# apache/yunikorn-k8shim

Measured on AMD Instinct MI355X. Metric: pod×node predicate evals/sec + decisions/sec, 50k nodes × 1M pods, higher is better.
Workload: dtype int64; 1 GPU; configs[2]: 50k nodes x 1M pods, NodeResourcesFit + TaintToleration + NodeAffinity; nodes_per_gpu=50000, total_nodes=50000, pods=1000000, templates=2000, pod_classes=2061, signature_planes=327, unique_requests=False, spread=False, gang_size=0, parallelism=single GPU

## Files before the change

yunikorn-k8shim_amd/csrc/engine/engine.hip:

```cpp
#include "../../../include/ykpred.h"

#include <hip/hip_runtime.h>
#include <dlfcn.h>
#include <rccl/rccl.h>

#include <algorithm>
#include <chrono>
#include <cstdio>
#include <cstdlib>
#include <cstring>
#include <mutex>
#include <string>
#include <map>
#include <unordered_map>
#include <vector>

#include "kernels.hip.h"
#include "ask_tasks.h"
#include "preempt_headroom_finish.h"

using ykk::i64;
using ykk::u64;

namespace {
// ... 205 lines not shown
  std::vector<int32_t> h_row_big;
  std::vector<int32_t> h_sorted_off;
  DevBuf d_sorted, d_sorted_off, d_ent_c;
  int sweep_min_run = 1;
  int sweep_groups = 0;
  bool sweep_ready = false;
  std::vector<int32_t> h_class_sweep;
  int sweep_rows[ykk::kMaxIdxRows] = {0, 0}, sweep_row_off[ykk::kMaxIdxRows + 1] = {0, 0, 0}, sweep_runs = 0;
  int index_rows_needed = 0;
  DevBuf d_agree;
  DevBuf d_query;
  DevBuf d_groups;
  DevBuf d_domain_head;
  DevBuf d_rc_req, d_rc_pods, d_rc_ports;
  int rc_tiers = 0;
  bool rc_ports = false;
  DevBuf d_vt_base, d_vt_tier_end, d_vt_cum, d_vt_ports;
  std::vector<int32_t> h_vt_base, h_vt_cap;
  int vt_tiers = 0;
  size_t vt_rows = 0;
  bool vt_ports = false;
  int64_t vt_max_cap = 0;
  DevBuf d_pround;
  DevBuf d_vfx_col, d_vfx_cum;
  int vfx_columns = -1;
  std::vector<uint8_t> vfx_stale;
  int64_t vfx_stale_nodes = 0;
  DevBuf d_pround_live;
  DevBuf d_bytes_gather;
  DevBuf d_topo_agree;
  u64 dict_digest = 0;
  int fuse_rows = 1;
  int fuse_wpl = 0;
  int fuse_count = 0, fuse_row_count = 0;
  bool fuse_ready = false;
  DevBuf d_fuse_rec;
  int fuse_combos = 0;
  int fuse_combine = 1;
  DevBuf d_fuse_combo_rec, d_fuse_combo;
  std::vector<uint8_t> h_class_fused;
  int run_decide = 1;
  int run_ranges = 0, n_decide_list = 0, run_decide_classes = -1;
  bool win_partial = false;
  DevBuf d_run_ranges, d_no_decide, d_glin_r;
  int class_runs = 1;
  int class_runs_min_rows = 16;
  int run_classes = 0, run_units = 0, run_rows = 0;
  DevBuf d_run_classes, d_run_units;
  DevBuf d_sweep_rows, d_sweep_runs, d_sweep_units;
  int sweep_units[ykk::kMaxIdxRows] = {0, 0}, sweep_unit_off[ykk::kMaxIdxRows + 1] = {0, 0, 0};
  DevBuf d_chunk_list_b0;
  int NCB0 = 0;
  DevBuf d_walk2_order, d_walk2_big, d_walk2_begin, d_walk2_len;
  int walk2_chunks = -1;
  DevBuf d_first_r;
  static constexpr bool decide_skip = true;
  DevBuf d_chunk_list_b;
  DevBuf d_slice_general;
  DevBuf d_slice_desc;
  DevBuf d_pfx_r;
  DevBuf d_idx_c;
  DevBuf d_win_r;
  int idx_stride = 0;
  DevBuf d_sig_tol, d_sig_tolflags, d_sig_ports, d_swanted;
  DevBuf d_sig_aff_flags, d_sig_aff_off, d_sig_aff_terms, d_sig_pre_off, d_sig_pre_terms;
  bool specs_set = false;

  int P = 0, C = 0, NC = 0;
  std::vector<int32_t> h_pod_spec, h_pod_pin;
  DevBuf d_pod_spec, d_pod_pin, d_pod_class;
  DevBuf d_class_sig, d_class_pin, d_class_first, d_class_word, d_chunk_class, d_chunk_begin, d_chunk_len, d_chunk_first, d_members;
  std::unordered_map<ClassKey, int32_t, ClassKeyHash> class_ids;
  std::vector<int32_t> h_pod_class, h_pod_slot;
  std::vector<int32_t> h_pod_row;
  int rows_total = 0, rows_a = 0, row_capacity = 0;
  DevBuf d_pod_row;
  bool bands_enabled = true;
  int band_steps = 0;
  int band_steps_now = 128;
  int round_batched = -1;
  int round_node_assume = 1;
  int round_prof = 0;
  int fail_after = 0;
  int sig_wpl = 0;
  int combine_slices = 1;
  int decide_groups_from = 16384;
  int early_counts = 1;
  int group_lds = -1;
  int group_scratch_mb = 256;
  int affinity_fill_waves = 0;
  int group_chunk_tasks = 0;
  int max_lds_bytes = 64 * 1024;
  int num_cus = 256;
  int n_bands = 0, n_band_steps = 0, n_classes_a = 0, n_fix_rows = 0;
  std::vector<int32_t> h_class_slot_a;
  DevBuf d_band_tab, d_class_rows_a, d_class_list_a, d_class_slot_a, d_fix_row, d_fix_slot, d_chunk_zone;
  DevBuf d_class_list_b;
  int n_classes_b = 0;
  std::vector<int32_t> h_ch_zone;
  std::vector<uint8_t> h_row_stale;
  std::vector<int32_t> h_class_sig, h_class_pin, h_class_first, h_class_live;
  std::vector<std::vector<int32_t>> h_class_chunks;
  std::vector<int32_t> h_members, h_ch_class, h_ch_begin, h_ch_len, h_ch_first;
  int patch_chunks = 0;
  bool rank_valid = false;
  uint64_t specs_version = 1, ranked_specs_version = 0, ranked_nodes_epoch = 0;
  unsigned ranked_pre = 0, ranked_filt = 0;
  bool ranked_has_first = false;
  DevBuf d_round;
  DevBuf d_fx_off, d_fx_cls, d_fx_cnt, d_fx_occ, d_sp_sig_of;
  uint64_t fx_version = 0;
  bool fx_contrib = false, fx_ports = false;
  std::vector<int32_t> h_fx_off;
  std::vector<int32_t> h_fx_cls;
  std::vector<int32_t> h_fx_cnt;
  std::vector<uint8_t> h_fx_occupies;
  DevBuf d_patches, d_rows, d_row_count, d_row_best;
  unsigned last_pre = 0, last_filt = 0;
  bool last_eval_valid = false;
  DevBuf d_class_count, d_class_best;
  bool pods_set = false, classes_dirty = true;
  int chunk_members = ykk::kChunkMembers;
  bool chunk_sorted = true;
  int combine_lds_bytes = 40000;

  DevBuf d_bitmap, d_counts, d_decisions, d_keys, d_scratch;
  void* last_bitmap = nullptr;
  int64_t last_bitmap_rows = 0;
  void *last_counts = nullptr, *last_decisions = nullptr, *last_keys = nullptr;

  hipStream_t aux_stream = nullptr;
  hipEvent_t ev_fork = nullptr, ev_planes = nullptr, ev_join = nullptr, ev_counts = nullptr, ev_zero = nullptr;
  hipStream_t peek_stream = nullptr;
  hipEvent_t ev_eval_done = nullptr;
  void* peek_pinned = nullptr;
  size_t peek_pinned_bytes = 0;

  struct GraphKey {
    uint64_t version;
    unsigned pre, filt, options;
    void *bitmap, *counts, *decisions, *keys;
    bool operator==(const GraphKey& o) const {
      return version == o.version && pre == o.pre && filt == o.filt && options == o.options && bitmap == o.bitmap && counts == o.counts &&
             decisions == o.decisions && keys == o.keys;
    }
  };
  std::vector<std::pair<GraphKey, hipGraphExec_t>> graphs;
  std::vector<GraphKey> seen;
  uint64_t tables_version = 1;
  bool graph_disabled = true;

  ncclComm_t comm = nullptr;
  int comm_rank = 0, comm_world = 1, node_offset = 0;
  int64_t round_exchanges = 0;
  void* h_round_pinned = nullptr;
  size_t h_round_pinned_bytes = 0;
  int64_t rounds_batched = 0, round_batched_asks = 0, round_batches = 0, rounds_sequential = 0, round_sequential_asks = 0;
  int forced_stride = 0;
  DevBuf d_gathered, d_gathered_map, d_xkey, d_xcand;
  bool last_has_keys = false;
  DevBuf d_class_rows_all, d_gathered_classes, d_class_rows_slot, d_class_sig_ident, d_expand_count, d_layout_hash, d_gathered_pod_class, d_row_pod;
  int ident_classes = 0;
  uint64_t layout_version = 1, layout_hashed_version = 0, layout_hash_value = 0, row_pod_version = 0;
  uint64_t ask_epoch = 1, hdr_epoch = 0;
  std::vector<uint64_t> hdr_cache;
  uint64_t nodes_epoch = 1, hist_epoch = 0;
  uint64_t bitmap_epoch = 0;

  int64_t n_full_evals = 0, n_node_patches = 0, n_row_patches = 0, n_queries = 0, n_gathers = 0, n_uploads = 0;

  hipEvent_t ev[2 * YKPRED_MAX_TIMED_KERNELS + 2]{};
  bool ev_ready = false;
  int timed = 0;
  const char* timed_name[YKPRED_MAX_TIMED_KERNELS]{};
  bool timing_valid = false;
};

namespace {

int fail(ykpred_engine* e, int code, const std::string& msg) {
  if (e) e->err = msg;
// ... 46 lines not shown
  t.KS = e->KS;
  t.domain = e->d_domain.as<int>();
  t.selcount = e->d_selcount.as<int>();
  t.KP = e->KP;
  t.ports = e->d_ports.as<u64>();
  return t;
}
ykk::SpreadSigs spread_sigs(const ykpred_engine* e) {
  ykk::SpreadSigs sp;
  sp.D = e->fam_spread.D;
  sp.c_off = e->d_sp_coff.as<int>();
  sp.c = e->d_sp_c.as<ykk::SpreadC>();
  sp.aff_sig = e->d_sp_aff.as<int>();
  sp.tol_sig = e->d_sp_tol.as<int>();
  sp.cnt = e->d_sp_cnt.as<int>();
  sp.present = e->d_sp_present.as<int>();
  sp.minv = e->d_sp_min.as<int>();
  return sp;
}
ykk::SpecTable spec_table(const ykpred_engine* e) {
  ykk::SpecTable s;
  s.R = e->R;
  s.KT = e->KT;
  s.W = e->W;
  s.req = e->d_sreq.as<i64>();
  s.tol = e->d_stol.as<u64>();
  s.flags = e->d_sflags.as<unsigned>();
  s.aff.flags = e->d_sflags.as<unsigned>();
  s.aff.term_off = e->d_aff_off.as<int>();
  s.aff.terms = e->d_aff_terms.as<u64>();
  s.aff.pre_off = e->d_pre_off.as<int>();
  s.aff.pre_terms = e->d_pre_terms.as<u64>();
  s.KP = e->KP;
  s.wanted_ports = e->d_swanted.as<u64>();
  s.spread_sig = e->d_spec_spread.as<int>();
  s.spread = spread_sigs(e);
  return s;
}

int build_classes(ykpred_engine* e, hipStream_t st) {
  e->tables_version++;
  const int P = e->P;
  auto& ids = e->class_ids;
  ids.clear();
  ids.reserve(1024);
  auto& pod_class = e->h_pod_class;
  pod_class.assign((size_t)P, 0);
  auto &class_sig = e->h_class_sig, &class_pin = e->h_class_pin, &class_size = e->h_class_live;
  class_sig.clear();
  class_pin.clear();
  class_size.clear();
  for (int p = 0; p < P; ++p) {
    int s = e->h_pod_spec[(size_t)p];
    ClassKey k{e->spec_sig_res[(size_t)s], e->spec_sig_tol[(size_t)s], e->spec_sig_aff[(size_t)s], e->spec_sig_spread[(size_t)s],
               e->h_pod_pin[(size_t)p]};
    auto it = ids.find(k);
    int32_t c;
    if (it == ids.end()) {
      c = (int32_t)class_pin.size();
      ids.emplace(k, c);
      class_sig.insert(class_sig.end(), {k.a, k.b, k.c, k.d});
      class_pin.push_back(k.pin);
      class_size.push_back(0);
    } else {
      c = it->second;
    }
    pod_class[(size_t)p] = c;
    class_size[(size_t)c]++;
  }
  const int C = (int)class_pin.size();
  std::vector<int32_t> class_off((size_t)C + 1, 0);
  for (int c = 0; c < C; ++c) class_off[(size_t)c + 1] = class_off[(size_t)c] + class_size[(size_t)c];
  auto& members = e->h_members;
  members.assign((size_t)P, 0);
  e->h_pod_slot.assign((size_t)P, 0);
  std::vector<int32_t> cursor(class_off.begin(), class_off.end() - 1);
  for (int p = 0; p < P; ++p) {
    int slot = cursor[(size_t)pod_class[(size_t)p]]++;
    members[(size_t)slot] = p;
    e->h_pod_slot[(size_t)p] = slot;
  }
  const long row_b = (long)e->row_stride * 8, win = (long)ykk::kBandGroups * 4096;
  const int KC = ykk::kBandClasses;
  auto piece_min_of = [&](int steps) { return (int)((double)steps * (4096.0 + (double)row_b) / (double)row_b / (double)(KC - 1) * 1.3) + 3; };
  int S = e->band_steps;
  if (S <= 0) {
    int s_min = 8;
    while (s_min < 128 && (long)s_min * 4096 < 5L * KC * row_b) s_min *= 2;
    auto coverage = [&](int steps) {
      const int need = 2 * piece_min_of(steps);
      long rows = 0;
      for (int c = 0; c < C; ++c)
        if (class_size[(size_t)c] >= need) rows += class_size[(size_t)c];
      return rows;
    };
    const long best = coverage(s_min);
    S = 128;
    while (S > s_min && (double)coverage(S) < 0.5 * (double)best) S /= 2;
  }
  while (S > 4 && (long)S * win / row_b >= (1L << 21)) S -= 4;
  e->band_steps_now = S;
  const int piece_min = piece_min_of(S);
  e->h_class_slot_a.assign((size_t)C, -1);
  e->h_pod_row.assign((size_t)P, -1);
  std::vector<ykk::BandEntry> band_tab;
  std::vector<int32_t> class_list_a, fix_row, fix_slot;
  int n_steps = 0, n_bands = 0, rows_a = 0;
  const bool geometry_ok = e->bands_enabled && e->N > 0 && (size_t)2 * KC * (size_t)row_b <= (size_t)std::min(ykk::kBandMaxLds, e->max_lds_bytes);
  if (geometry_ok) {
    long rows_needed = 0;
    for (int c = 0; c < C; ++c)
      if (class_size[(size_t)c] >= 2 * piece_min) {
        e->h_class_slot_a[(size_t)c] = (int32_t)class_list_a.size();
        class_list_a.push_back(c);
        rows_needed += class_size[(size_t)c];
      }
    if (rows_needed < (long)S * win / row_b / 4) {
      class_list_a.clear();
      std::fill(e->h_class_slot_a.begin(), e->h_class_slot_a.end(), -1);
    }
  }
  if (!class_list_a.empty()) {
    struct Piece {
      int32_t x, s, slot;
    };
    size_t ci = 0;
    int32_t left = class_size[(size_t)class_list_a[0]], taken = 0;
    bool ok = true;
    std::vector<uint64_t> keys;
    std::vector<Piece> pieces;
    int band = 0;
    while (ci < class_list_a.size() && ok) {
      const long band_rows = (long)S * win / row_b;
      long remaining = left;
      for (size_t k = ci + 1; k < class_list_a.size() && remaining <= band_rows; ++k) remaining += class_size[(size_t)class_list_a[k]];
      const long s_lo = (long)band * S;
      long band_steps_now = S;
      if (remaining + piece_min + 2 < band_rows) {
        band_steps_now = ((remaining + piece_min + 2) * row_b + win - 1) / win;
        band_steps_now = std::min<long>(S, std::max<long>(4, (band_steps_now + 3) / 4 * 4));
      }
      const long s_hi = s_lo + band_steps_now;
      const long r_lo = (s_lo * win + row_b - 1) / row_b, r_hi = (s_hi * win + row_b - 1) / row_b;
      keys.resize((size_t)(r_hi - r_lo));
      for (size_t i = 0; i < keys.size(); ++i) {
        const long r = r_lo + (long)i, start = r * row_b;
        keys[i] = ((uint64_t)(start % win) << 42) | ((uint64_t)(start / win) << 21) | (uint64_t)i;
      }
      std::sort(keys.begin(), keys.end());
      pieces.clear();
      size_t pos = 0;
      const size_t cap = keys.size();
      while (pos < cap && ci < class_list_a.size()) {
        const size_t room = cap - pos;
        if (room < (size_t)piece_min) break;
        size_t take = std::min<size_t>((size_t)left, room);
        if ((size_t)left > take && (size_t)left - take < (size_t)piece_min) {
          if (take < (size_t)piece_min + (size_t)piece_min) break;
          take = (size_t)left - (size_t)piece_min;
        }
        const int c = class_list_a[ci];
        const uint64_t k0 = keys[pos];
        pieces.push_back({(int32_t)(k0 >> 42), (int32_t)((k0 >> 21) & 0x1fffff), (int32_t)ci});
        for (size_t i = 0; i < take; ++i) {
          const long r = r_lo + (long)(keys[pos + i] & 0x1fffff);
          const int p = members[(size_t)(class_off[(size_t)c] + taken + (int32_t)i)];
          e->h_pod_row[(size_t)p] = (int32_t)r;
        }
        pos += take;
        taken += (int32_t)take;
        left -= (int32_t)take;
        if (left == 0) {
          ++ci;
          taken = 0;
          if (ci < class_list_a.size()) left = class_size[(size_t)class_list_a[ci]];
        }
      }
      for (int b = 0; b < ykk::kBandGroups && ok; ++b) {
        ykk::BandEntry be{};
        for (int i = 0; i < KC; ++i) be.slot[i] = pieces.empty() ? 0 : pieces[0].slot;
        for (int i = 0; i < KC - 1; ++i) {
          be.xb[i] = 0x7fffffff;
          be.sb[i] = 0;
        }
        const long x_lo = std::max<long>(0, (long)b * 4096 - row_b + 1), x_hi = (long)(b + 1) * 4096;
        size_t ia = 0;
        for (size_t i = 0; i < pieces.size(); ++i)
          if ((long)pieces[i].x < x_lo) ia = i;
        if (!pieces.empty()) be.slot[0] = pieces[ia].slot;
        int n = 1;
        for (size_t i = ia + 1; i < pieces.size() && (long)pieces[i].x < x_hi; ++i) {
          if (n >= KC) {
            ok = false;
            break;
          }
          be.slot[n] = pieces[i].slot;
          be.xb[n - 1] = pieces[i].x;
          be.sb[n - 1] = pieces[i].s;
          ++n;
        }
        for (int i = n; i < KC; ++i) be.slot[i] = be.slot[n - 1];
        be.n = n;
        be.steps = (int32_t)band_steps_now;
        be.first_step = (int32_t)s_lo;
        band_tab.push_back(be);
      }
      ++band;
      n_steps = (int)s_hi;
      rows_a = (int)r_hi;
      if (band_steps_now < S) break;
    }
    if (ci < class_list_a.size()) ok = false;
    if (!ok) {
      class_list_a.clear();
      std::fill(e->h_class_slot_a.begin(), e->h_class_slot_a.end(), -1);
      std::fill(e->h_pod_row.begin(), e->h_pod_row.end(), -1);
      band_tab.clear();
      n_steps = n_bands = rows_a = 0;
    } else {
      n_bands = band;
      std::vector<int32_t> row_slot((size_t)rows_a, -1);
      for (int c : class_list_a)
        for (int i = class_off[(size_t)c]; i < class_off[(size_t)c + 1]; ++i) row_slot[(size_t)e->h_pod_row[(size_t)members[(size_t)i]]] = e->h_class_slot_a[(size_t)c];
      for (long s1 = 1; s1 <= n_steps; ++s1) {
        const long r = (s1 * win - 1) / row_b;
        if (r * row_b + row_b > s1 * win && r < rows_a && row_slot[(size_t)r] >= 0) {
          fix_row.push_back((int32_t)r);
          fix_slot.push_back(row_slot[(size_t)r]);
        }
      }
    }
  }
  int next_row = rows_a;
  e->h_class_sweep.assign((size_t)C, 0);
  e->sweep_ready = false;
  e->sweep_runs = 0;
  e->run_ranges = 0;
  e->walk2_chunks = -1;
  e->index_rows_needed = e->index_rows;
  for (int b = 0; b < ykk::kMaxIdxRows; ++b) e->sweep_rows[b] = 0;
  {
    std::vector<int32_t> order_b;
    for (int c = 0; c < C; ++c)
      if (e->h_class_slot_a[(size_t)c] < 0) order_b.push_back(c);
    auto key = [&](int32_t c, int f) { return class_sig[(size_t)c * 4 + (size_t)f]; };
    const int R1 = 1 + e->R, big_mask = (1 << ykk::kRowBigShift) - 1;
    bool sweep_possible = e->sweep_min_run > 0 && e->n_big > 0 && !e->h_res_rows.empty() && (int)e->h_sorted_off.size() == e->n_big + 1;
    for (int b = 0; sweep_possible && b < e->n_big; ++b)
      sweep_possible = e->h_sorted_off[(size_t)b + 1] - e->h_sorted_off[(size_t)b] < (1 << 26);
    std::vector<int32_t> cand_big, cand_slot, cand_pos;
    if (sweep_possible) {
      cand_big.assign((size_t)C, -1);
      cand_slot.assign((size_t)C, -1);
      cand_pos.assign((size_t)C, -1);
      for (int32_t c : order_b) {
        const int sr = key(c, 0);
        if (class_size[(size_t)c] != 1 || class_pin[(size_t)c] != -1 || sr < 0 || (size_t)(sr + 1) * (size_t)R1 > e->h_res_rows.size()) continue;
        const int32_t* rr = e->h_res_rows.data() + (size_t)sr * (size_t)R1;
        int np = 0, ni = 0, prow = -1, irow = -1;
        for (int k = 0; k < R1; ++k) {
          const int r = rr[k];
          if (r < 0) continue;
          if (r >> ykk::kRowBigShift) {
            if (ni == 0) irow = r;
            ++ni;
          } else {
            if (np == 1) prow = r;
            ++np;
          }
        }
        if (ni != 1 || np < 1 || np > 2) continue;
        const int slot = np == 2 ? prow : 0;
        const int pos = e->h_row_pos[(size_t)(irow & big_mask)];
        if (pos < 0) continue;
        cand_big[(size_t)c] = (irow >> ykk::kRowBigShift) - 1;
        cand_slot[(size_t)c] = slot;
        cand_pos[(size_t)c] = pos;
      }
    }
    auto is_cand = [&](int32_t c) { return sweep_possible && cand_slot[(size_t)c] >= 0; };
    std::vector<int32_t> run_slots;
    const bool runs_possible = e->class_runs != 0 && !e->h_res_rows.empty() && e->h_stage_rows.size() < 255;
    if (runs_possible) {
      run_slots.assign((size_t)C, -1);
      const int n_stage = (int)e->h_stage_rows.size();
      for (int32_t c : order_b) {
        const int sr = key(c, 0);
        if (class_pin[(size_t)c] != -1 || sr < 0 || (size_t)(sr + 1) * (size_t)R1 > e->h_res_rows.size()) continue;
        const int32_t* rr = e->h_res_rows.data() + (size_t)sr * (size_t)R1;
        int n = 0, packed = 0;
        bool ok = true;
        for (int k = 0; k < R1 && ok; ++k) {
          const int r = rr[k];
          if (r <= 0) continue;
          if (r >> ykk::kRowBigShift) ok = false;
          int slot = -1;
          for (int q = 0; q < n_stage && ok; ++q)
            if (e->h_stage_rows[(size_t)q] == r) slot = q;
          if (slot < 0 || n >= 4) ok = false;
          else packed |= slot << (8 * n++);
        }
        if (!ok) continue;
        for (; n < 4; ++n) packed |= n_stage << (8 * n);
        run_slots[(size_t)c] = packed;
      }
    }
    auto kind_of = [&](int32_t c) { return is_cand(c) ? 2 : (runs_possible && run_slots[(size_t)c] >= 0 ? 1 : 0); };
    std::vector<uint8_t> tail((size_t)C, 0);
    {
      struct SigKey {
        int32_t a, t, s, k, b, p;
        bool operator==(const SigKey& o) const { return a == o.a && t == o.t && s == o.s && k == o.k && b == o.b && p == o.p; }
      };
      struct SigHash {
        size_t operator()(const SigKey& q) const {
          uint64_t h = 0x9e3779b97f4a7c15ull;
          for (int32_t v : {q.a, q.t, q.s, q.k, q.b, q.p}) h = (h ^ (uint64_t)(uint32_t)v) * 0x100000001b3ull;
          return (size_t)h;
        }
      };
      std::unordered_map<SigKey, long, SigHash> rows_of_sig;
      auto sig_key = [&](int32_t c, int kind) {
        return SigKey{key(c, 2), key(c, 1), key(c, 3), kind, kind == 2 ? cand_big[(size_t)c] : 0, kind == 2 ? cand_slot[(size_t)c] : 0};
      };
      for (int32_t c : order_b) {
        const int kind = kind_of(c);
        if (kind) rows_of_sig[sig_key(c, kind)] += class_size[(size_t)c];
      }
      for (int32_t c : order_b) {
        const int kind = kind_of(c);
        tail[(size_t)c] = kind == 0 || rows_of_sig[sig_key(c, kind)] < (kind == 1 ? (long)e->class_runs_min_rows : (long)e->sweep_min_run);
      }
    }
    std::sort(order_b.begin(), order_b.end(), [&](int32_t x, int32_t y) {
      if (tail[(size_t)x] != tail[(size_t)y]) return tail[(size_t)x] < tail[(size_t)y];
      if (key(x, 2) != key(y, 2)) return key(x, 2) < key(y, 2);
      if (key(x, 1) != key(y, 1)) return key(x, 1) < key(y, 1);
      if (key(x, 3) != key(y, 3)) return key(x, 3) < key(y, 3);
      const int kx = kind_of(x), ky = kind_of(y);
      if (kx != ky) return kx < ky;
      if (kx == 2) {
        if (cand_big[(size_t)x] != cand_big[(size_t)y]) return cand_big[(size_t)x] < cand_big[(size_t)y];
        if (cand_slot[(size_t)x] != cand_slot[(size_t)y]) return cand_slot[(size_t)x] < cand_slot[(size_t)y];
        if (cand_pos[(size_t)x] != cand_pos[(size_t)y]) return cand_pos[(size_t)x] < cand_pos[(size_t)y];
        return x < y;
      }
      if (key(x, 0) != key(y, 0)) return key(x, 0) < key(y, 0);
      return x < y;
    });
    std::vector<int32_t> first_row_of((size_t)C, -1);
    for (int32_t c : order_b) {
      first_row_of[(size_t)c] = next_row;
      for (int i = class_off[(size_t)c]; i < class_off[(size_t)c + 1]; ++i) e->h_pod_row[(size_t)members[(size_t)i]] = next_row++;
    }
    e->n_classes_b = (int)order_b.size();
    TRY(upload(e, e->d_class_list_b, order_b.data(), order_b.size(), st));
    std::vector<ykk::SweepRun> runs;
    e->run_classes = e->run_units = e->run_rows = 0;
    if (runs_possible) {
      std::vector<ykk::RunClass> rcs;
      std::vector<int32_t> starts;
      for (size_t i = 0; i < order_b.size();) {
        const int32_t c = order_b[i];
        if (kind_of(c) != 1) {
          ++i;
          continue;
        }
        size_t j = i;
        long rows_in_run = 0;
        while (j < order_b.size() && kind_of(order_b[j]) == 1 && key(order_b[j], 2) == key(c, 2) && key(order_b[j], 1) == key(c, 1) &&
               key(order_b[j], 3) == key(c, 3)) {
          rows_in_run += class_size[(size_t)order_b[j]];
          ++j;
        }
        if (rows_in_run >= e->class_runs_min_rows) {
          ykk::SweepRun run{};
          run.st = key(c, 1), run.sa = key(c, 2), run.ss = key(c, 3), run.prow = 0;
          runs.push_back(run);
          for (size_t k = i; k < j; ++k) {
            const int32_t m = order_b[k];
            ykk::RunClass rc{};
            rc.cls = m, rc.dest0 = first_row_of[(size_t)m], rc.len = class_size[(size_t)m], rc.slots = run_slots[(size_t)m], rc.run = (int32_t)runs.size() - 1;
            rcs.push_back(rc);
            starts.push_back(k == i ? 1 : 0);
            e->h_class_sweep[(size_t)m] = 1;
          }
        }
        i = j;
      }
      if (!rcs.empty()) {
        const int n = (int)rcs.size();
        auto cost = [&](int i) { return (long)rcs[(size_t)i].len + ykk::kRunsClassCost + (starts[(size_t)i] ? ykk::kSweepRunCost : 0); };
        long total = 0;
        for (int i = 0; i < n; ++i) total += cost(i);
        const int want = std::max(1, std::min(n / 2, 2 * e->num_cus * ykk::kRunsWaves * 8));
        std::vector<int32_t> units;
        long acc = 0;
        for (int i = 0; i < n; ++i) {
          if ((long)units.size() < want && acc * want >= (long)units.size() * total) units.push_back(i);
          acc += cost(i);
        }
        e->run_units = (int)units.size();
        units.push_back(n);
        e->run_classes = n;
        for (const ykk::RunClass& rc : rcs) e->run_rows += rc.len;
        TRY(upload(e, e->d_run_classes, rcs.data(), rcs.size(), st));
        TRY(upload(e, e->d_run_units, units.data(), units.size(), st));
      }
    }
    if (sweep_possible) {
      std::vector<int32_t> rows_of[ykk::kMaxIdxRows];
      for (size_t i = 0; i < order_b.size();) {
        const int32_t c = order_b[i];
        if (!is_cand(c)) {
          ++i;
          continue;
        }
        size_t j = i + 1;
        while (j < order_b.size() && is_cand(order_b[j]) && key(order_b[j], 2) == key(c, 2) && key(order_b[j], 1) == key(c, 1) &&
               key(order_b[j], 3) == key(c, 3) && cand_big[(size_t)order_b[j]] == cand_big[(size_t)c] &&
               cand_slot[(size_t)order_b[j]] == cand_slot[(size_t)c])
          ++j;
        if ((int)(j - i) >= e->sweep_min_run) {
          const int big = cand_big[(size_t)c];
          ykk::SweepRun run{};
          run.st = key(c, 1), run.sa = key(c, 2), run.ss = key(c, 3), run.prow = cand_slot[(size_t)c];
          const int32_t id = (int32_t)runs.size();
          runs.push_back(run);
          for (size_t k = i; k < j; ++k) {
            const int32_t m = order_b[k];
            e->h_class_sweep[(size_t)m] = 1;
            rows_of[big].insert(rows_of[big].end(), {m, first_row_of[(size_t)m], cand_pos[(size_t)m], id});
          }
        }
        i = j;
      }
      e->sweep_runs = (int)runs.size();
      std::vector<int32_t> all_rows, all_units;
      std::vector<ykk::RunRange> ranges;
// ... 92 lines not shown
      for (int c = 0; c < C; ++c)
        if (key(c, 2) >= 0 && key(c, 2) < e->fam_aff.D) users[(size_t)key(c, 2)]++;
      std::vector<ykk::FuseRec> recs;
      for (int32_t c : order_b) {
        const int sa = key(c, 2), sr = key(c, 0), stl = key(c, 1);
        if (!tail[(size_t)c] || e->h_class_sweep[(size_t)c] || class_size[(size_t)c] < 1 || class_pin[(size_t)c] != -1 || key(c, 3) >= 0) continue;
        if (sa < 0 || sa >= e->fam_aff.D || sr < 0 || (size_t)(sr + 1) * (size_t)R1 > e->h_res_rows.size()) continue;
        ykk::FuseRec rec{};
        rec.cls = c, rec.dest = first_row_of[(size_t)c], rec.len = class_size[(size_t)c];
        rec.row[rec.n++] = (2 << ykk::kFuseFamShift) | sa;
        if (stl >= 0) rec.row[rec.n++] = (1 << ykk::kFuseFamShift) | stl;
        bool ok = true;
        for (int k = 0; k < R1 && ok; ++k) {
          const int r = e->h_res_rows[(size_t)sr * (size_t)R1 + (size_t)k];
          if (r < 0) continue;
          if ((r >> ykk::kRowBigShift) || rec.n >= 8) ok = false;
          else rec.row[rec.n++] = r;
        }
        if (!ok) continue;
        recs.push_back(rec);
        e->h_class_fused[(size_t)c] = 1;
        e->fuse_count++;
        e->fuse_row_count += rec.len;
      }
      e->fuse_combos = 0;
      if (e->fuse_count > 0) {
        std::unordered_map<uint64_t, int32_t> combo_of;
        std::vector<ykk::FuseRec> combo_recs;
        std::vector<int32_t> combo_ix(recs.size(), -1);
        for (size_t i = 0; i < recs.size(); ++i) {
          const int32_t c = recs[i].cls;
          const uint64_t k2 = ((uint64_t)(uint32_t)key(c, 1) << 32) | (uint32_t)key(c, 0);
          auto it = combo_of.find(k2);
          if (it == combo_of.end()) {
            it = combo_of.emplace(k2, (int32_t)combo_recs.size()).first;
            ykk::FuseRec cr{};
            cr.cls = 0, cr.dest = it->second, cr.len = 1;
            for (int k = 1; k < recs[i].n; ++k) cr.row[cr.n++] = recs[i].row[k];
            combo_recs.push_back(cr);
          }
          combo_ix[i] = it->second;
        }
        bool combine = e->fuse_combine != 0 && combo_recs.size() * 4 <= recs.size() && combo_recs.size() <= 16384;
        for (const ykk::FuseRec& cr : combo_recs) combine = combine && cr.n >= 1;
        if (combine) {
          for (size_t i = 0; i < recs.size(); ++i) {
            recs[i].n = 2;
            recs[i].row[1] = (3 << ykk::kFuseFamShift) | combo_ix[i];
          }
          e->fuse_combos = (int)combo_recs.size();
          TRY(upload(e, e->d_fuse_combo_rec, combo_recs.data(), combo_recs.size(), st));
          HIPCHK(e->d_fuse_combo.ensure((size_t)e->fuse_combos * (size_t)e->row_stride * sizeof(u64)));
        }
        TRY(upload(e, e->d_fuse_rec, recs.data(), recs.size(), st));
        e->fuse_ready = true;
      }
      if (getenv("YKPRED_TRACE_RUNS")) {
        long t_cls = 0, t_rows = 0, t_single = 0, t_single_shared = 0, t_single_big = 0, t_single_spread = 0, t_pinned = 0;
        for (int32_t c : order_b) {
          if (!tail[(size_t)c] || e->h_class_sweep[(size_t)c] || e->h_class_fused[(size_t)c]) continue;
          ++t_cls, t_rows += class_size[(size_t)c];
          if (class_size[(size_t)c] == 1) {
            ++t_single;
            const int sa = key(c, 2);
            if (sa >= 0 && sa < e->fam_aff.D && users[(size_t)sa] != 1) ++t_single_shared;
            if (key(c, 3) >= 0) ++t_single_spread;
            if (class_pin[(size_t)c] != -1) ++t_pinned;
            const int sr = key(c, 0);
            if (sr >= 0)
              for (int k = 0; k < R1; ++k)
                if (e->h_res_rows[(size_t)sr * (size_t)R1 + (size_t)k] > 0 && (e->h_res_rows[(size_t)sr * (size_t)R1 + (size_t)k] >> ykk::kRowBigShift)) { ++t_single_big; break; }
          }
        }
        fprintf(stderr, "fused: %d classes, %d rows, %d combinations; chunk writers keep %ld classes / %ld rows of zone B (%ld single-row: %ld share their affinity signature, %ld with an index row, %ld spread, %ld pinned)\n",
                e->fuse_count, e->fuse_row_count, e->fuse_combos, t_cls, t_rows, t_single, t_single_shared, t_single_big, t_single_spread, t_pinned);
      }
    }
  }
  e->rows_total = next_row;
  e->rows_a = rows_a;
  e->n_bands = n_bands;
  e->n_band_steps = n_steps;
  e->n_classes_a = (int)class_list_a.size();
  e->n_fix_rows = (int)fix_row.size();
  if (e->row_capacity && e->rows_total > e->row_capacity)
    return fail(e, YKPRED_E_INVALID, "the bitmap needs more rows than ykpred_set_row_capacity allows");
  const int cm = e->chunk_members;
  struct Chunk {
    int32_t cls, begin, len, first, first_row;
  };
  std::vector<Chunk> chunks;
  for (int c = 0; c < C; ++c)
    for (int b = class_off[(size_t)c]; b < class_off[(size_t)c + 1]; b += cm)
      chunks.push_back({c, b, std::min(cm, class_off[(size_t)c + 1] - b), b == class_off[(size_t)c] ? 1 : 0, e->h_pod_row[(size_t)members[(size_t)b]]});
  if (e->chunk_sorted)
    std::stable_sort(chunks.begin(), chunks.end(), [](const Chunk& x, const Chunk& y) { return x.first_row < y.first_row; });
  auto &ch_class = e->h_ch_class, &ch_begin = e->h_ch_begin, &ch_len = e->h_ch_len, &ch_first = e->h_ch_first;
  ch_class.clear();
  ch_begin.clear();
  ch_len.clear();
  ch_first.clear();
  e->h_ch_zone.clear();
  e->h_class_chunks.assign((size_t)C, {});
  for (const Chunk& k : chunks) {
    e->h_class_chunks[(size_t)k.cls].push_back((int32_t)ch_class.size());
    ch_class.push_back(k.cls);
    ch_begin.push_back(k.begin);
    ch_len.push_back(k.len);
    ch_first.push_back(k.first);
    e->h_ch_zone.push_back(e->h_class_slot_a[(size_t)k.cls] >= 0 ? 1 : (e->h_class_sweep[(size_t)k.cls] ? 2 : (e->h_class_fused[(size_t)k.cls] ? 3 : 0)));
  }
  std::vector<int32_t> chunk_list_b;
  for (size_t k = 0; k < e->h_ch_zone.size(); ++k)
    if (e->h_ch_zone[k] != 1) chunk_list_b.push_back((int32_t)k);
  e->NCB = (int)chunk_list_b.size();
  {
    std::vector<int32_t> chunk_list_b0;
    for (size_t k = 0; k < e->h_ch_zone.size(); ++k)
      if (e->h_ch_zone[k] == 0) chunk_list_b0.push_back((int32_t)k);
    e->NCB0 = (int)chunk_list_b0.size();
    TRY(upload(e, e->d_chunk_list_b0, chunk_list_b0.data(), chunk_list_b0.size(), st));
  }
  e->h_class_first.assign((size_t)C, -1);
  for (int c = 0; c < C; ++c) e->h_class_first[(size_t)c] = members[(size_t)class_off[(size_t)c]];
  std::vector<int32_t> member_rows((size_t)P);
  for (int i = 0; i < P; ++i) member_rows[(size_t)i] = e->h_pod_row[(size_t)members[(size_t)i]];
  e->h_row_stale.assign((size_t)P, 0);
  e->C = C;
  e->NC = (int)ch_class.size();
  e->patch_chunks = 0;
  TRY(upload(e, e->d_pod_class, pod_class.data(), pod_class.size(), st));
  TRY(upload(e, e->d_class_sig, class_sig.data(), class_sig.size(), st));
  TRY(upload(e, e->d_class_pin, class_pin.data(), class_pin.size(), st));
  TRY(upload(e, e->d_class_first, e->h_class_first.data(), e->h_class_first.size(), st));
  TRY(upload(e, e->d_members, member_rows.data(), member_rows.size(), st));
  TRY(upload(e, e->d_pod_row, e->h_pod_row.data(), e->h_pod_row.size(), st));
  TRY(upload(e, e->d_chunk_zone, e->h_ch_zone.data(), e->h_ch_zone.size(), st));
  TRY(upload(e, e->d_chunk_list_b, chunk_list_b.data(), chunk_list_b.size(), st));
  TRY(upload(e, e->d_band_tab, band_tab.data(), band_tab.size(), st));
  TRY(upload(e, e->d_class_list_a, class_list_a.data(), class_list_a.size(), st));
  TRY(upload(e, e->d_class_slot_a, e->h_class_slot_a.data(), e->h_class_slot_a.size(), st));
  TRY(upload(e, e->d_fix_row, fix_row.data(), fix_row.size(), st));
  TRY(upload(e, e->d_fix_slot, fix_slot.data(), fix_slot.size(), st));
  HIPCHK(e->d_class_rows_a.ensure((size_t)std::max<size_t>(class_list_a.size(), 1) * (size_t)e->row_stride * sizeof(u64)));
  TRY(upload(e, e->d_chunk_class, ch_class.data(), ch_class.size(), st));
  TRY(upload(e, e->d_chunk_begin, ch_begin.data(), ch_begin.size(), st));
  TRY(upload(e, e->d_chunk_len, ch_len.data(), ch_len.size(), st));
  TRY(upload(e, e->d_chunk_first, ch_first.data(), ch_first.size(), st));
  HIPCHK(e->d_class_count.ensure((size_t)std::max(C, 1) * sizeof(int)));
  HIPCHK(e->d_class_best.ensure((size_t)std::max(C, 1) * sizeof(int)));
  HIPCHK(hipStreamSynchronize(st));
  e->classes_dirty = false;
  e->layout_version++;
  e->last_eval_valid = false;
  return YKPRED_OK;
}

int ensure_planes(ykpred_engine* e, hipStream_t st) {
  int rows = 0;
  for (Family* f : {&e->fam_res, &e->fam_spread, &e->fam_tol, &e->fam_aff}) {
    f->base = rows;
    rows += std::max(f->D, 1);
  }
  size_t need = ((size_t)rows * (size_t)e->row_stride + 64) * sizeof(u64);
  for (DevBuf* b : {&e->planes_canon, &e->planes_ranked}) {
    if (b->cap < need || e->plane_rows_alloc != rows) {
      e->tables_version++;
      HIPCHK(b->ensure(need));
      HIPCHK(hipMemsetAsync(b->p, 0, need, st));
    }
  }
  e->plane_rows_alloc = rows;
  size_t base_need = (size_t)(64 * (e->W + e->KT + e->KP) + 2) * (size_t)e->row_stride * sizeof(u64);
  for (DevBuf* b : {&e->base_canon, &e->base_ranked}) {
    if (b->cap < base_need) {
      e->tables_version++;
      HIPCHK(b->ensure(base_need));
      HIPCHK(hipMemsetAsync(b->p, 0, base_need, st));
    }
  }
  return YKPRED_OK;
}

int build_spread_tables(ykpred_engine* e, hipStream_t st) {
  e->tables_version++;
  std::vector<int32_t> coff{0}, aff, tol;
  std::vector<ykk::SpreadC> rows;
  int64_t cells = 0;
  for (size_t d = 0; d < e->spread_sig.size(); ++d) {
    for (const ykpred_spread_t& c : e->spread_sig[d]) {
      if (c.topology_key < 0 || c.topology_key >= e->KD || c.selector_class >= e->KS)
        return fail(e, YKPRED_E_INVALID, "spread constraint references a topology key / selector class outside the node table");
      ykk::SpreadC r;
      r.kd = c.topology_key;
      r.ks = c.selector_class;
      r.max_skew = c.max_skew;
      r.min_domains = c.min_domains;
      r.self_match = c.self_match;
      r.flags = c.flags;
      r.kind = c.kind;
      r.dom_size = (size_t)c.topology_key < e->h_domain_sizes.size() ? e->h_domain_sizes[(size_t)c.topology_key] : 0;
      r.cnt_off = (int)cells;
      cells += r.dom_size;
      if (cells > 0x7fffffff) return fail(e, YKPRED_E_UNSUPPORTED, "spread histograms exceed 2^31 cells");
      rows.push_back(r);
    }
    coff.push_back((int32_t)rows.size());
    aff.push_back(e->spread_sig_aff[d]);
    tol.push_back(e->spread_sig_tol[d]);
  }
  e->spread_constraints = (int)rows.size();
  e->spread_cells = cells;
  TRY(upload(e, e->d_sp_coff, coff.data(), coff.size(), st));
  TRY(upload(e, e->d_sp_c, rows.data(), rows.size(), st));
  TRY(upload(e, e->d_sp_aff, aff.data(), aff.size(), st));
  TRY(upload(e, e->d_sp_tol, tol.data(), tol.size(), st));
  {
    std::vector<int32_t> sig_of;
    for (size_t d = 0; d < e->spread_sig.size(); ++d) sig_of.insert(sig_of.end(), e->spread_sig[d].size(), (int32_t)d);
    sig_of.resize(std::max<size_t>(rows.size(), 1), 0);
    TRY(upload(e, e->d_sp_sig_of, sig_of.data(), sig_of.size(), st));
  }
  HIPCHK(e->d_sp_cnt.ensure((size_t)std::max<int64_t>(cells, 1) * sizeof(int)));
  HIPCHK(e->d_sp_present.ensure((size_t)std::max<int64_t>(cells, 1) * sizeof(int)));
  HIPCHK(e->d_sp_min.ensure((size_t)std::max(e->spread_constraints, 1) * sizeof(int)));
  HIPCHK(hipStreamSynchronize(st));
// ... 253 lines not shown

#define YK_SERIALISE(eng) \
  std::unique_lock<std::recursive_mutex> engine_lock; \
  if (eng) engine_lock = std::unique_lock<std::recursive_mutex>((eng)->mu)

extern "C" {

int32_t ykpred_abi_version(void) { return YKPRED_ABI_VERSION; }

const char* ykpred_last_error(const ykpred_engine_t* e) { return e ? e->err.c_str() : g_create_error.c_str(); }

int32_t ykpred_create(const ykpred_config_t* cfg, ykpred_engine_t** out) {
  if (!cfg || !out) {
    g_create_error = "null argument";
    return YKPRED_E_INVALID;
  }
  if (cfg->abi_version != YKPRED_ABI_VERSION) {
    g_create_error = "ABI version mismatch";
    return YKPRED_E_INVALID;
  }
  if (cfg->num_resources < 3 || cfg->num_resources > ykk::kMaxR || cfg->taint_words < 1 || cfg->taint_words > ykk::kMaxKT ||
      cfg->label_words < 1 || cfg->label_words > ykk::kMaxWTotal) {
    g_create_error = "config out of range: need 3<=R<=8, 1<=KT<=4, 1<=W<=32";
    return YKPRED_E_UNSUPPORTED;
  }
  if (cfg->topology_keys < 0 || cfg->topology_keys > ykk::kMaxKD || cfg->selector_classes < 0 || cfg->selector_classes > 4096 ||
      cfg->port_words < 0 || cfg->port_words > ykk::kMaxKP) {
    g_create_error = "config out of range: need 0<=KD<=8 topology keys, 0<=KS<=4096 selector classes, 0<=KP<=4 port words";
    return YKPRED_E_UNSUPPORTED;
  }
  int ndev = 0;
  hipError_t s = hipGetDeviceCount(&ndev);
  if (s != hipSuccess || ndev <= 0) {
    g_create_error = std::string("no HIP device: ") + hipGetErrorString(s) + " (libykpred has no CPU fallback)";
    return YKPRED_E_DEVICE;
  }
  if (cfg->device < 0 || cfg->device >= ndev) {
    g_create_error = "device ordinal out of range";
    return YKPRED_E_INVALID;
  }
  s = hipSetDevice(cfg->device);
  if (s != hipSuccess) {
    g_create_error = std::string("hipSetDevice: ") + hipGetErrorString(s);
    return YKPRED_E_DEVICE;
  }
  auto* e = new ykpred_engine();
  e->cfg = *cfg;
  e->R = cfg->num_resources;
  e->KT = cfg->taint_words;
  e->W = cfg->label_words;
  e->KD = cfg->topology_keys;
  e->KS = cfg->selector_classes;
  e->KP = cfg->port_words;
  if (cfg->reserved[0] >= 1 && cfg->reserved[0] <= ykk::kChunkMembers) e->chunk_members = cfg->reserved[0];
  e->chunk_sorted = cfg->reserved[1] != 1;
  if (cfg->reserved[2] > 0 && cfg->reserved[2] <= 160 * 1024) e->combine_lds_bytes = cfg->reserved[2];
  if (cfg->reserved[2] < 0) e->combine_lds_bytes = 0;
  if (cfg->reserved[4] > 0) e->walk_rows = cfg->reserved[4];
  if (cfg->reserved[5] > 0) e->wave_combine_below = cfg->reserved[5];
  if (cfg->reserved[5] < 0) e->wave_combine_below = 0;
  if (cfg->reserved[6] < 0) e->bands_enabled = false;
  if (cfg->reserved[6] > 0) e->band_steps = std::min(256, std::max(4, (cfg->reserved[6] + 3) / 4 * 4));
  e->graph_disabled = cfg->reserved[3] != 1;
  {
    int lds = 0;
    if (hipDeviceGetAttribute(&lds, hipDeviceAttributeMaxSharedMemoryPerBlock, cfg->device) == hipSuccess && lds > 0) e->max_lds_bytes = lds;
    int cus = 0;
    if (hipDeviceGetAttribute(&cus, hipDeviceAttributeMultiprocessorCount, cfg->device) == hipSuccess && cus > 0) e->num_cus = cus;
  }
  if (const char* tune = getenv("YKPRED_TUNE")) {
    std::string text(tune);
    size_t at = 0;
    while (at < text.size()) {
      size_t stop = text.find(',', at);
      if (stop == std::string::npos) stop = text.size();
      const std::string item = text.substr(at, stop - at);
      at = stop + 1;
      if (item.empty()) continue;
      const size_t eq = item.find('=');
      const std::string key = item.substr(0, eq);
      const int val = eq == std::string::npos ? 1 : atoi(item.c_str() + eq + 1);
      if (key == "walk_rows") e->walk_rows = std::max(val, 1);
      else if (key == "sig_wpl") e->sig_wpl = val;
      else if (key == "combine_slices") e->combine_slices = val;
      else if (key == "decide_groups_from") e->decide_groups_from = val;
      else if (key == "graph") e->graph_disabled = val != 1;
      else if (key == "early_counts") e->early_counts = val;
      else if (key == "band_steps") {
        e->bands_enabled = val >= 0;
        e->band_steps = val > 0 ? std::min(256, std::max(4, (val + 3) / 4 * 4)) : 0;
      } else if (key == "chunk_members") e->chunk_members = std::min(std::max(val, 1), (int)ykk::kChunkMembers);
      else if (key == "wave_combine_below") e->wave_combine_below = std::max(val, 0);
      else if (key == "fail_after") e->fail_after = std::max(val, 0);
      else if (key == "round_prof") e->round_prof = val;
      else if (key == "round_batched") e->round_batched = val;
      else if (key == "round_node_assume") e->round_node_assume = val;
      else if (key == "sweep_min_run") e->sweep_min_run = std::max(val, 0);
      else if (key == "sweep_groups") e->sweep_groups = std::max(val, 0);
      else if (key == "class_runs") e->class_runs = val;
      else if (key == "run_decide") e->run_decide = val;
      else if (key == "fuse_rows") e->fuse_rows = val;
      else if (key == "fuse_wpl") e->fuse_wpl = val;
      else if (key == "fuse_combine") e->fuse_combine = val;
      else if (key == "class_runs_min_rows") e->class_runs_min_rows = std::max(val, 1);
      else if (key == "group_lds") e->group_lds = val;
      else if (key == "group_scratch_mb") e->group_scratch_mb = std::max(val, 0);
      else if (key == "group_chunk_tasks") e->group_chunk_tasks = std::max(val, 0);
      else if (key == "affinity_fill_waves") e->affinity_fill_waves = val;
      else {
        g_create_error = "YKPRED_TUNE: unknown key '" + key + "'";
        delete e;
        return YKPRED_E_INVALID;
      }
    }
  }
  s = hipStreamCreateWithFlags(&e->own_stream, hipStreamNonBlocking);
  if (s != hipSuccess) {
    g_create_error = std::string("hipStreamCreate: ") + hipGetErrorString(s);
    delete e;
    return YKPRED_E_DEVICE;
  }
  {
    int lo = 0, hi = 0;
    (void)hipDeviceGetStreamPriorityRange(&lo, &hi);
    if (hipStreamCreateWithPriority(&e->aux_stream, hipStreamNonBlocking, hi) != hipSuccess)
      (void)hipStreamCreateWithFlags(&e->aux_stream, hipStreamNonBlocking);
  }
  if (hipStreamCreateWithFlags(&e->peek_stream, hipStreamNonBlocking) != hipSuccess) e->peek_stream = nullptr;
  (void)hipEventCreateWithFlags(&e->ev_eval_done, hipEventDisableTiming);
  (void)hipEventCreateWithFlags(&e->ev_fork, hipEventDisableTiming);
  (void)hipEventCreateWithFlags(&e->ev_join, hipEventDisableTiming);
  (void)hipEventCreateWithFlags(&e->ev_planes, hipEventDisableTiming);
  (void)hipEventCreateWithFlags(&e->ev_counts, hipEventDisableTiming);
  (void)hipEventCreateWithFlags(&e->ev_zero, hipEventDisableTiming);
  for (auto& ev : e->ev) (void)hipEventCreate(&ev);
  e->ev_ready = true;
  *out = e;
  return YKPRED_OK;
}

void ykpred_destroy(ykpred_engine_t* e) {
  if (!e) return;
  (void)hipSetDevice(e->cfg.device);
  (void)hipDeviceSynchronize();
  if (e->comm) (void)rccl()->CommDestroy(e->comm);
  e->comm = nullptr;
  for (DevBuf* b : {&e->d_gathered, &e->d_gathered_map, &e->d_xkey, &e->d_xcand}) b->release();
  for (auto& g : e->graphs) (void)hipGraphExecDestroy(g.second);
  e->graphs.clear();
  for (DevBuf* b : {&e->d_alloc, &e->d_req, &e->d_allowed, &e->d_count, &e->d_nflags, &e->d_taints, &e->d_labels, &e->d_domain, &e->d_selcount, &e->d_ports, &e->d_sig_ports, &e->d_swanted,
                    &e->d_sp_cnt_prev, &e->d_sp_present_prev, &e->d_sp_min_prev, &e->d_sig_changed, &e->d_class_dirty,
                    &e->d_spec_spread, &e->d_sp_coff, &e->d_sp_c, &e->d_sp_aff, &e->d_sp_tol, &e->d_sp_cnt, &e->d_sp_present, &e->d_sp_min,
                    &e->planes_canon, &e->planes_ranked, &e->base_canon, &e->base_ranked, &e->d_rankbuf, &e->d_score, &e->d_key,
                    &e->d_rank, &e->d_perm, &e->d_sreq, &e->d_stol, &e->d_sflags, &e->d_aff_off, &e->d_aff_terms, &e->d_pre_off,
                    &e->d_pre_terms, &e->d_dim_val, &e->d_dim_order, &e->d_dim_chunk_dim, &e->d_dim_chunk_begin, &e->d_dim_chunk_len,
                    &e->d_res_rows, &e->d_big_dim, &e->d_walk_big, &e->d_walk_begin, &e->d_walk_len, &e->d_sfree_c, &e->d_pmask_c,
                    &e->d_sfree_r, &e->d_pmask_r, &e->d_rbits_c, &e->d_sorted, &e->d_sorted_off, &e->d_ent_c, &e->d_agree, &e->d_topo_agree, &e->d_bytes_gather, &e->d_fuse_rec, &e->d_fuse_combo_rec, &e->d_fuse_combo, &e->d_run_ranges, &e->d_no_decide, &e->d_glin_r, &e->d_run_classes, &e->d_run_units, &e->d_sweep_rows, &e->d_sweep_runs, &e->d_sweep_units, &e->d_chunk_list_b0, &e->d_walk2_order, &e->d_walk2_big, &e->d_walk2_begin, &e->d_walk2_len, &e->d_idx_c, &e->d_win_r, &e->d_pfx_r, &e->d_slice_desc, &e->d_slice_general, &e->d_chunk_list_b, &e->d_first_r, &e->d_sig_tol, &e->d_sig_tolflags, &e->d_sig_aff_flags, &e->d_sig_aff_off,
                    &e->d_sig_aff_terms, &e->d_sig_pre_off, &e->d_sig_pre_terms, &e->d_pod_spec, &e->d_pod_pin, &e->d_pod_class,
                    &e->d_class_sig, &e->d_class_pin, &e->d_class_first, &e->d_class_word, &e->d_chunk_class, &e->d_chunk_begin, &e->d_chunk_len, &e->d_chunk_first,
                    &e->d_pod_row, &e->d_band_tab, &e->d_class_rows_a, &e->d_class_list_a, &e->d_class_slot_a, &e->d_fix_row, &e->d_fix_slot, &e->d_chunk_zone,
                    &e->d_members, &e->d_patches, &e->d_rows, &e->d_row_count, &e->d_row_best, &e->d_class_count, &e->d_class_best, &e->d_bitmap, &e->d_counts, &e->d_decisions, &e->d_keys, &e->d_scratch,
                    &e->d_member_key, &e->d_name_rank, &e->d_member_tie, &e->d_class_rows_all, &e->d_gathered_classes, &e->d_class_rows_slot,
                    &e->d_class_sig_ident, &e->d_expand_count, &e->d_layout_hash, &e->d_gathered_pod_class, &e->d_row_pod,
                    &e->d_round, &e->d_fx_off, &e->d_fx_cls, &e->d_fx_cnt, &e->d_fx_occ, &e->d_sp_sig_of, &e->d_class_list_b, &e->d_gathered, &e->d_gathered_map,
                    &e->d_xkey, &e->d_xcand, &e->d_query, &e->d_groups, &e->d_domain_head, &e->d_rc_req, &e->d_rc_pods, &e->d_rc_ports,
                    &e->d_vt_base, &e->d_vt_tier_end, &e->d_vt_cum, &e->d_vt_ports, &e->d_pround})
    b->release();
  if (e->ev_ready)
    for (auto& ev : e->ev) (void)hipEventDestroy(ev);
  if (e->ev_fork) (void)hipEventDestroy(e->ev_fork);
  if (e->ev_join) (void)hipEventDestroy(e->ev_join);
  if (e->ev_planes) (void)hipEventDestroy(e->ev_planes);
  if (e->ev_counts) (void)hipEventDestroy(e->ev_counts);
  if (e->ev_zero) (void)hipEventDestroy(e->ev_zero);
  if (e->h_round_pinned) (void)hipHostFree(e->h_round_pinned);
  if (e->ev_eval_done) (void)hipEventDestroy(e->ev_eval_done);
  if (e->peek_pinned) (void)hipHostFree(e->peek_pinned);
  if (e->peek_stream) (void)hipStreamDestroy(e->peek_stream);
  if (e->aux_stream) (void)hipStreamDestroy(e->aux_stream);
  if (e->own_stream) (void)hipStreamDestroy(e->own_stream);
  delete e;
}

int32_t ykpred_set_nodes(ykpred_engine_t* e, const ykpred_nodes_t* n) {
  YK_SERIALISE(e);
  Range roctx_range("ykpred:upload_nodes");
  if (e) e->n_uploads++;
  if (e) e->tables_version++;
  if (e) e->nodes_epoch++;
  if (e) e->ask_epoch++;
  if (e) e->last_eval_valid = false;
  if (!e || !n || n->count < 0) return fail(e, YKPRED_E_INVALID, "set_nodes: bad argument");
  if (n->count > 0 && (!n->allocatable || !n->requested || !n->allowed_pods || !n->pod_count || !n->flags || !n->taint_bits ||
                       !n->label_bits))
    return fail(e, YKPRED_E_INVALID, "set_nodes: null column");
  if ((e->KD > 0 && (!n->domain_sizes || (n->count > 0 && !n->domain_id))) || (e->KS > 0 && n->count > 0 && !n->selector_count))
    return fail(e, YKPRED_E_INVALID, "set_nodes: topology / selector columns missing (config has KD/KS > 0)");
  if (e->KP > 0 && n->count > 0 && !n->port_bits) return fail(e, YKPRED_E_INVALID, "set_nodes: port_bits missing (config has KP > 0)");
  HIPCHK(hipSetDevice(e->cfg.device));
  hipStream_t st = e->own_stream;
  e->rank_valid = false;
  const size_t N = (size_t)n->count;
  TRY(upload(e, e->d_alloc, n->allocatable, N * (size_t)e->R, st));
  TRY(upload(e, e->d_req, n->requested, N * (size_t)e->R, st));
  TRY(upload(e, e->d_allowed, n->allowed_pods, N, st));
  TRY(upload(e, e->d_count, n->pod_count, N, st));
  TRY(upload(e, e->d_nflags, n->flags, N, st));
  TRY(upload(e, e->d_taints, n->taint_bits, N * (size_t)e->KT, st));
  TRY(upload(e, e->d_labels, n->label_bits, N * (size_t)e->W, st));
  TRY(upload(e, e->d_domain, n->domain_id, N * (size_t)e->KD, st));
  TRY(upload(e, e->d_selcount, n->selector_count, N * (size_t)e->KS, st));
  TRY(upload(e, e->d_ports, n->port_bits, N * (size_t)e->KP, st));
  e->has_name_rank = n->name_rank != nullptr && N > 0;
  if (e->has_name_rank) TRY(upload(e, e->d_name_rank, n->name_rank, N, st));
  HIPCHK(e->d_member_tie.ensure(std::max<size_t>(N, 1) * sizeof(int)));
  for (int k = 0; k < ykk::kMaxKT; ++k) e->taint_used[k] = 0;
  for (int k = 0; k < e->KT; ++k)
    for (size_t i = 0; i < N; ++i) e->taint_used[k] |= n->taint_bits[(size_t)k * N + i];
  e->h_domain_sizes.assign(n->domain_sizes, n->domain_sizes + e->KD);
  e->spread_dirty = true;
  HIPCHK(e->d_score.ensure(N * sizeof(double)));
  HIPCHK(e->d_key.ensure(N * sizeof(u64)));
  HIPCHK(e->d_rank.ensure(N * sizeof(int)));
  HIPCHK(e->d_perm.ensure(N * sizeof(int)));
  HIPCHK(e->d_rankbuf.ensure((3 * (size_t)ykk::kRankBuckets + 1 + N) * sizeof(int)));
  HIPCHK(e->d_member_key.ensure(N * sizeof(u64)));
  HIPCHK(hipStreamSynchronize(st));
  if (e->N != n->count) {
    e->planes_canon.release();
    e->planes_ranked.release();
    e->base_canon.release();
    e->base_ranked.release();
    e->rc_tiers = 0;
    e->vt_tiers = 0;
    e->vfx_columns = -1;
  }
  e->N = n->count;
  e->row_words = (e->N + 63) / 64;
  e->row_stride = std::max(16, (e->row_words + 15) / 16 * 16);
  if (e->forced_stride) {
    if (e->forced_stride < e->row_stride) return fail(e, YKPRED_E_INVALID, "set_nodes: ykpred_set_row_stride is smaller than this shard needs");
    e->row_stride = e->forced_stride;
  }
// ... 523 lines not shown
                     use_run_decide ? e->d_no_decide.as<int>() : nullptr};
  ykk::Planes pc{res_on ? o_res.canon : nullptr, o_tol.canon, aff_on ? o_aff.canon : nullptr, spread_on ? o_spread.canon : nullptr,
                 e->row_stride, e->d_res_rows.as<int>(), 1 + e->R, e->d_idx_c.as<unsigned char>(), e->idx_stride, e->d_pmask_c.as<u64>(), e->row_words,
                 nullptr, 0, 0, 0, 0, 0, nullptr, nullptr, nullptr, nullptr, nullptr};
  int* first_r = nullptr;
  if ((a->options & (YKPRED_OUT_DECISIONS | YKPRED_OUT_DECISION_KEYS)) && e->decide_skip) {
    HIPCHK(e->d_first_r.ensure((size_t)std::max(e->plane_rows_alloc, 1) * sizeof(int)));
    first_r = e->d_first_r.as<int>();
  }
  if (want_dec && res_on && e->n_big > 0 && !fit_error) HIPCHK(e->d_pfx_r.ensure((size_t)e->n_big * (size_t)std::max(e->row_words, 1) * sizeof(i64)));
  ykk::Planes pr = ranked_planes_of(e, pre, filt, spread_on, first_r != nullptr);
  pc.n_big = pr.n_big;
  pc.rbits = e->d_rbits_c.as<u64>();
  const int pin_on = ((filt & YKPRED_PLUGIN_NODE_NAME) ? 1 : 0) | (spread_err ? 2 : 0);
  hipStream_t sb = e->aux_stream;

  if (want_dec) {
    HIPCHK(hipEventRecord(e->ev_fork, st));
    HIPCHK(hipStreamWaitEvent(sb, e->ev_fork, 0));
    if (zero_counts_beside) {
      HIPCHK(hipMemsetAsync(e->d_class_count.p, 0, (size_t)e->C * sizeof(int), sb));
      HIPCHK(hipEventRecord(e->ev_zero, sb));
    }
    if (first_r) HIPCHK(hipMemsetAsync(first_r, 0x7f, (size_t)std::max(e->plane_rows_alloc, 1) * sizeof(int), sb));
    tm.begin(sb);
    hipLaunchKernelGGL(ykk::k_score, dim3((unsigned)nblk_nodes), dim3(ykk::kBlock), 0, sb, nt, e->d_score.as<double>(), e->d_key.as<u64>());
    tm.end(sb, "k_score");
    int* hist = e->d_rankbuf.as<int>();
    int* bucket_off = hist + ykk::kRankBuckets;
    int* cursor = bucket_off + ykk::kRankBuckets + 1;
    int* members = cursor + ykk::kRankBuckets;
    HIPCHK(hipMemsetAsync(hist, 0, ykk::kRankBuckets * sizeof(int), sb));
    tm.begin(sb);
    hipLaunchKernelGGL(ykk::k_rank_hist, dim3((unsigned)nblk_nodes), dim3(ykk::kBlock), 0, sb, N, e->d_score.as<double>(), hist);
    hipLaunchKernelGGL(ykk::k_rank_scan, dim3(1), dim3(ykk::kRankBuckets), 0, sb, hist, bucket_off, cursor);
    hipLaunchKernelGGL(ykk::k_rank_fill, dim3((unsigned)nblk_nodes), dim3(ykk::kBlock), 0, sb, N, e->d_score.as<double>(), e->d_key.as<u64>(),
                       e->has_name_rank ? e->d_name_rank.as<int>() : (const int*)nullptr, cursor, members, e->d_member_tie.as<int>(),
                       e->d_member_key.as<u64>());
    hipLaunchKernelGGL(ykk::k_rank_final, dim3((unsigned)ykk::kRankBuckets), dim3(ykk::kBlock), 0, sb, bucket_off, members,
                       e->d_member_tie.as<int>(), e->d_member_key.as<u64>(), e->d_rank.as<int>(), e->d_perm.as<int>());
    tm.end(sb, "k_rank");
  }
  auto base_of = [&](DevBuf& buf) {
    ykk::BasePlanes bp;
    bp.req = buf.as<u64>();
    bp.taint = bp.req + (size_t)64 * e->W * e->row_stride;
    bp.port = bp.taint + (size_t)64 * e->KT * e->row_stride;
    bp.unsched = bp.port + (size_t)64 * e->KP * e->row_stride;
    bp.exists = bp.unsched + e->row_stride;
    bp.stride = e->row_stride;
    return bp;
  };
  auto launch_dictionary_planes = [&](hipStream_t s, const int* perm, bool ranked, const char* base_name, const char* sig_name, bool base_done = false) -> int {
    ykk::BasePlanes bp = base_of(ranked ? e->base_ranked : e->base_canon);
    if (!base_done) {
      tm.begin(s);
      hipLaunchKernelGGL(ykk::k_base_planes, dim3((unsigned)(e->W + e->KT + e->KP + 1), wgroups), dim3(ykk::kBlock), 0, s, nt, perm, bp,
                         e->row_words);
      tm.end(s, base_name);
    }
    ykk::SigPlaneArgs sa{};
    sa.base = bp;
    sa.tol = o_tol;
    sa.aff = o_aff;
    if (ranked) {
      sa.tol.canon = o_tol.ranked;
      sa.aff.canon = o_aff.ranked;
      sa.tol.first = first_r ? first_r + e->fam_tol.base : nullptr;
      sa.aff.first = first_r ? first_r + e->fam_aff.base : nullptr;
    }
    if (!aff_on) sa.aff.D = 0;
    sa.sig_tol = e->d_sig_tol.as<u64>();
    sa.sig_tolflags = e->d_sig_tolflags.as<unsigned>();
    sa.sig_ports = e->d_sig_ports.as<u64>();
    sa.KP = e->KP;
    for (int k = 0; k < ykk::kMaxKT; ++k) sa.taint_used[k] = e->taint_used[k];
    sa.affs = as;
    sa.KT = e->KT;
    sa.W = e->W;
    sa.pre_mask = pre;
    sa.filt_mask = filt;
    sa.n_words = e->row_words;
    tm.begin(s);
    const int wpl = e->sig_wpl > 0 ? e->sig_wpl : (e->row_words >= 4 * ykk::kWave ? 4 : (e->row_words >= 2 * ykk::kWave ? 2 : 1));
    const unsigned chunks = std::max((unsigned)((std::max(sa.tol.D, sa.aff.D) + ykk::kBitSigsPerBlock - 1) / ykk::kBitSigsPerBlock), 1u);
    const unsigned ygroups = (unsigned)((e->row_words + ykk::kBlock * wpl - 1) / (ykk::kBlock * wpl));
    if (wpl >= 4)
      hipLaunchKernelGGL(ykk::k_sig_planes<4>, dim3(chunks, ygroups, 2u), dim3(ykk::kBlock), 0, s, sa);
    else if (wpl >= 2)
      hipLaunchKernelGGL(ykk::k_sig_planes<2>, dim3(chunks, ygroups, 2u), dim3(ykk::kBlock), 0, s, sa);
    else
      hipLaunchKernelGGL(ykk::k_sig_planes<1>, dim3(chunks, ygroups, 2u), dim3(ykk::kBlock), 0, s, sa);
    tm.end(s, sig_name);
    return YKPRED_OK;
  };
  if (want_dec) TRY(launch_dictionary_planes(sb, e->d_perm.as<int>(), true, "k_base_planes(ranked)", "k_sig_planes(ranked)"));
  auto ranked_walk = [](const int* perm) { return perm != nullptr; };
  auto launch_ballot_planes = [&](hipStream_t s, const int* perm, const char* name, bool with_base = false) {
    ykk::PlaneArgs pa{};
    pa.perm = perm;
    pa.res = o_res;
    pa.spread = o_spread;
    if (perm && first_r) {
      pa.res.first = first_r + e->fam_res.base;
      pa.spread.first = first_r + e->fam_spread.base;
    }
    if (!spread_on) pa.spread.D = 0;
    pa.dims = ykk::DimPlanes{e->d_dim_val.as<i64>(), e->d_dim_order.as<int>(), e->d_dim_chunk_dim.as<int>(), e->d_dim_chunk_begin.as<int>(),
                             e->d_dim_chunk_len.as<int>(), res_on ? e->dim_chunks : 0};
    pa.spreads = spread_sigs(e);
    pa.fit_error = fit_error;
    pa.n_words = e->row_words;
    pa.spread_en = pts_en ? 1 : 0;
    pa.ipa_en = ipa_en ? 1 : 0;
    unsigned xchunks = std::max((unsigned)pa.dims.n_chunks, sig_chunks(pa.spread.D));
    tm.begin(s);
    if (with_base) {
      xchunks = std::max(xchunks, (unsigned)(e->W + e->KT + e->KP + 1));
      hipLaunchKernelGGL(ykk::k_node_planes, dim3(std::max(xchunks, 1u), wgroups, 3u), dim3(ykk::kBlock), 0, s, nt, pa,
                         base_of(perm ? e->base_ranked : e->base_canon));
    } else {
      hipLaunchKernelGGL(ykk::k_planes, dim3(std::max(xchunks, 1u), wgroups, spread_on ? 2u : 1u), dim3(ykk::kBlock), 0, s, nt, pa);
    }
    tm.end(s, name);
    if (res_on && e->n_big > 0 && !fit_error) {
      const bool ranked = perm != nullptr;
      ykk::DimWalk dw{e->d_dim_val.as<i64>(), e->d_dim_order.as<int>(), e->d_big_dim.as<int>(), e->d_walk_big.as<int>(), e->d_walk_begin.as<int>(),
                      e->d_walk_len.as<int>(), (ranked ? e->d_sfree_r : e->d_sfree_c).as<i64>(), (ranked ? e->d_pmask_r : e->d_pmask_c).as<u64>(),
                      e->n_big, e->walk_chunks, e->row_words, ranked ? nullptr : e->d_rbits_c.as<u64>(),
                      (!ranked && sweep_rows_on) ? e->d_ent_c.as<unsigned>() : nullptr, e->d_sorted.as<i64>(), e->d_sorted_off.as<int>(),
                      (ranked && use_run_decide) ? e->d_glin_r.as<unsigned>() : nullptr};
      tm.begin(s);
      hipLaunchKernelGGL(ykk::k_dim_sort, dim3((unsigned)e->n_big, wgroups), dim3(ykk::kBlock), 0, s, nt, perm, dw);
      tm.end(s, ranked ? "k_dim_sort(ranked)" : "k_dim_sort");
      tm.begin(s);
      const unsigned walk_gy = (unsigned)((e->row_words + ykk::kBlock * ykk::kWalkWords - 1) / (ykk::kBlock * ykk::kWalkWords));
      const dim3 walk_grid((unsigned)e->walk_chunks, walk_gy);
      if (!ranked && use_sweep && e->walk2_chunks >= 0) {
        if (e->walk2_chunks > 0) {
          ykk::DimWalk dw2 = dw;
          dw2.order = e->d_walk2_order.as<int>();
          dw2.chunk_big = e->d_walk2_big.as<int>();
          dw2.chunk_begin = e->d_walk2_begin.as<int>();
          dw2.chunk_len = e->d_walk2_len.as<int>();
          dw2.n_chunks = e->walk2_chunks;
          hipLaunchKernelGGL(ykk::k_dim_walk, dim3((unsigned)e->walk2_chunks, walk_gy), dim3(ykk::kBlock), 0, s, dw2, e->d_idx_c.as<unsigned char>(), e->idx_stride);
        }
      } else if (!ranked) {
        hipLaunchKernelGGL(ykk::k_dim_walk, walk_grid, dim3(ykk::kBlock), 0, s, dw, e->d_idx_c.as<unsigned char>(), e->idx_stride);
      } else {
        hipLaunchKernelGGL(ykk::k_dim_prefix_max, dim3((unsigned)e->n_big), dim3(ykk::kPfxBlock), 0, s, dw, e->d_pfx_r.as<i64>());
        if (use_run_decide) {
          if (e->walk2_chunks > 0) {
            ykk::DimWalk dw2 = dw;
            dw2.order = e->d_walk2_order.as<int>();
            dw2.chunk_big = e->d_walk2_big.as<int>();
            dw2.chunk_begin = e->d_walk2_begin.as<int>();
            dw2.chunk_len = e->d_walk2_len.as<int>();
            dw2.n_chunks = e->walk2_chunks;
            hipLaunchKernelGGL(ykk::k_dim_walk_window<8>, dim3((unsigned)e->walk2_chunks, walk_gy), dim3(ykk::kBlock), 0, s, dw2, e->d_pfx_r.as<i64>(), e->d_win_r.as<unsigned char>());
          }
        } else {
          hipLaunchKernelGGL(ykk::k_dim_walk_window<ykk::kWalkBatch>, walk_grid, dim3(ykk::kBlock), 0, s, dw, e->d_pfx_r.as<i64>(), e->d_win_r.as<unsigned char>());
        }
      }
      tm.end(s, ranked ? "k_dim_walk(ranked)" : "k_dim_walk");
    } else if (res_on && e->n_big > 0) {
      if (!ranked_walk(perm)) (void)hipMemsetAsync(e->d_idx_c.p, 64, (size_t)e->fam_res.D * (size_t)e->idx_stride, s);
      (void)hipMemsetAsync((ranked_walk(perm) ? e->d_pmask_r : e->d_pmask_c).p, 0, (size_t)e->n_big * (size_t)e->row_words * 65 * sizeof(u64), s);
      if (!ranked_walk(perm)) (void)hipMemsetAsync(e->d_rbits_c.p, 0, (size_t)e->n_big * (size_t)e->row_words * ykk::kRankBits * sizeof(u64), s);
    }
  };
  const bool fused_planes = res_on || spread_on;
  if (fused_planes) launch_ballot_planes(st, nullptr, "k_planes+k_base_planes", true);
  TRY(launch_dictionary_planes(st, nullptr, false, "k_base_planes", "k_sig_planes", fused_planes));
  if (want_dec) {
    HIPCHK(hipEventRecord(e->ev_planes, st));
    HIPCHK(hipStreamWaitEvent(sb, e->ev_planes, 0));
    const int ballot_rows = e->fam_tol.base;
    if (ballot_rows <= ykk::kManySigs && e->n_big == 0) {
      tm.begin(sb);
      hipLaunchKernelGGL(ykk::k_permute_planes, dim3(sig_chunks(ballot_rows), wgroups), dim3(ykk::kBlock), 0, sb, N, e->d_perm.as<int>(),
                         e->planes_canon.as<u64>(), e->planes_ranked.as<u64>(), e->row_stride, ballot_rows, e->row_words, first_r);
      tm.end(sb, "k_permute_planes");
    } else if (res_on || spread_on) {
      launch_ballot_planes(sb, e->d_perm.as<int>(), "k_planes(ranked)");
    }
    if (use_run_decide) {
      tm.begin(sb);
      hipLaunchKernelGGL(ykk::k_run_decide, dim3((unsigned)((e->run_ranges + ykk::kWavesPerBlock - 1) / ykk::kWavesPerBlock)), dim3(ykk::kBlock), 0, sb, pr,
                         e->d_sweep_runs.as<ykk::SweepRun>(), e->d_run_ranges.as<ykk::RunRange>(), e->run_ranges, e->d_sweep_rows.as<ykk::SweepRow>(),
                         e->d_glin_r.as<unsigned>(), e->d_sorted.as<i64>(), e->d_sorted_off.as<int>(), e->d_perm.as<int>(), e->row_words, N, pin_on,
                         e->d_class_best.as<int>());
      tm.end(sb, "k_run_decide");
    }
    tm.begin(sb);
    const int n_decide = use_run_decide ? e->n_decide_list : e->C;
    if (n_decide == 0) {
    } else if (n_decide >= e->decide_groups_from) {
      const int per_block = ykk::kWavesPerBlock * ykk::kDecideGroups;
      hipLaunchKernelGGL(ykk::k_decide_groups, dim3((unsigned)((n_decide + per_block - 1) / per_block)), dim3(ykk::kBlock), 0, sb, ct, pr, n_decide,
                         e->row_words, e->d_perm.as<int>(), e->d_rank.as<int>(), pin_on, e->d_class_best.as<int>());
    } else {
      hipLaunchKernelGGL(ykk::k_decide, dim3((unsigned)((n_decide + ykk::kWavesPerBlock - 1) / ykk::kWavesPerBlock)), dim3(ykk::kBlock), 0, sb, ct,
                         pr, n_decide, e->row_words, e->d_perm.as<int>(), e->d_rank.as<int>(), pin_on, e->d_class_best.as<int>(), n_decide <= 4096 ? 1 : 0);
    }
    tm.end(sb, "k_decide");
  }
  const bool skip_combine = a->options & YKPRED_EVAL_SKIP_BITMAP;
  const bool dirty_only = a->options & YKPRED_EVAL_DIRTY_CLASSES;
  const int* class_dirty = nullptr;
  if (!skip_combine && dirty_only) {
    HIPCHK(e->d_class_dirty.ensure((size_t)std::max(e->C, 1) * sizeof(int)));
    hipLaunchKernelGGL(ykk::k_mark_dirty_classes, dim3((unsigned)((e->C + ykk::kBlock - 1) / ykk::kBlock)), dim3(ykk::kBlock), 0, st, e->C,
                       e->d_class_sig.as<int>(), e->d_sig_changed.as<int>(), e->d_class_dirty.as<int>(), e->d_class_count.as<int>());
    class_dirty = e->d_class_dirty.as<int>();
  }
  const bool small_chunks = (long)e->NC * e->wave_combine_below > (long)P;
  const bool counts_early = e->early_counts != 0 && !skip_combine && !dirty_only && e->n_classes_a > 0 && e->patch_chunks == 0 && !small_chunks && e->n_classes_b <= 16384;
  bool scattered = false;
  if (!skip_combine && !dirty_only && !counts_early) {
    if (zero_counts_beside) HIPCHK(hipStreamWaitEvent(st, e->ev_zero, 0));
    else HIPCHK(hipMemsetAsync(e->d_class_count.p, 0, (size_t)e->C * sizeof(int), st));
  }
  if (!skip_combine) {
    int tpg = ykk::kBlock;
    while (tpg > ykk::kWave && (tpg / 2) * 2 >= e->row_stride) tpg /= 2;
    const int seg = tpg * ykk::kCombineUnroll * 2;
    const bool listed = !dirty_only && e->patch_chunks == 0;
    const bool short_list = use_sweep && (fuse_on || e->fuse_count == 0);
    const int* chunk_list = listed ? (short_list ? e->d_chunk_list_b0 : e->d_chunk_list_b).as<int>() : nullptr;
    const int n_run = listed ? (short_list ? e->NCB0 : e->NCB) : e->NC;
    dim3 grid((unsigned)std::max(n_run, 1), (unsigned)((e->row_stride + seg - 1) / seg));
    hipStream_t sz = st;
    if (!dirty_only && e->n_classes_a > 0) {
      tm.begin(st);
      const int n_counted_b = counts_early ? e->n_classes_b : 0;
      hipLaunchKernelGGL(ykk::k_class_rows, dim3((unsigned)((e->n_classes_a + n_counted_b + ykk::kWavesPerBlock - 1) / ykk::kWavesPerBlock)), dim3(ykk::kBlock), 0, st,
                         ct, pc, e->d_class_list_a.as<int>(), e->n_classes_a, e->row_words, e->row_stride, pin_on, e->d_class_rows_a.as<u64>(),
                         e->d_class_count.as<int>(), (const int*)nullptr, e->d_class_list_b.as<int>(), n_counted_b);
      tm.end(st, "k_class_rows");
      if (counts_early && want_dec) {
        HIPCHK(hipEventRecord(e->ev_counts, st));
        HIPCHK(hipStreamWaitEvent(sb, e->ev_counts, 0));
        tm.begin(sb);
        hipLaunchKernelGGL(ykk::k_scatter, dim3((unsigned)((P + ykk::kBlock - 1) / ykk::kBlock)), dim3(ykk::kBlock), 0, sb, P,
                           e->d_pod_class.as<int>(), e->d_class_count.as<int>(), e->d_class_best.as<int>(), e->d_key.as<u64>(),
                           want_cnt ? (int*)e->last_counts : nullptr, (int*)e->last_decisions, want_keys ? (i64*)e->last_keys : nullptr);
        tm.end(sb, "k_scatter");
        scattered = true;
      }
      const size_t lds_bytes = (size_t)2 * ykk::kBandClasses * (size_t)e->row_stride * sizeof(u64);
      if (lds_bytes > 64 * 1024)
        HIPCHK(hipFuncSetAttribute((const void*)ykk::k_expand_bands, hipFuncAttributeMaxDynamicSharedMemorySize, (int)lds_bytes));
      tm.begin(st);
      hipLaunchKernelGGL(ykk::k_expand_bands, dim3((unsigned)ykk::kBandGroups), dim3(ykk::kBandBlock), lds_bytes, st, bitmap,
                         e->d_class_rows_a.as<u64>(), e->d_band_tab.as<ykk::BandEntry>(), e->n_bands, e->row_stride);
      if (e->n_fix_rows > 0 && !counts_early)
        hipLaunchKernelGGL(ykk::k_fix_rows, dim3((unsigned)e->n_fix_rows), dim3(ykk::kBlock), 0, st, bitmap, e->d_class_rows_a.as<u64>(),
                           e->d_fix_row.as<int>(), e->d_fix_slot.as<int>(), e->n_fix_rows, e->row_stride);
      tm.end(st, "k_expand_bands");
    }
    if (use_sweep && e->run_classes > 0) {
      ykk::WalkStage rstage{};
      rstage.n = (int)e->h_stage_rows.size();
      for (int k = 0; k < rstage.n; ++k) rstage.row[k] = e->h_stage_rows[(size_t)k];
      const int its = (e->row_stride + ykk::kWave - 1) / ykk::kWave;
      int segs = (its + ykk::kWalkMaxIt - 1) / ykk::kWalkMaxIt, nit = (its + segs - 1) / segs;
      while (nit > 1 && ykk::runs_lds_bytes(rstage.n, nit) > (size_t)e->max_lds_bytes) {
        ++segs;
        nit = (its + segs - 1) / segs;
      }
      const int n_long = segs - (nit * segs - its);
      const size_t lds = ykk::runs_lds_bytes(rstage.n, nit);
      const int per_cu = lds * 2 <= (size_t)e->max_lds_bytes ? 2 : 1;
      const int groups = std::max(1, std::min(per_cu * e->num_cus, (e->run_units + ykk::kRunsWaves - 1) / ykk::kRunsWaves));
      tm.begin(sz);
      auto launch_runs = [&](auto kernel) -> int {
        if (lds > 64 * 1024) HIPCHK(hipFuncSetAttribute((const void*)kernel, hipFuncAttributeMaxDynamicSharedMemorySize, (int)lds));
        hipLaunchKernelGGL(kernel, dim3((unsigned)groups, (unsigned)segs), dim3(ykk::kRunsThreads), lds, sz, pc, e->d_run_classes.as<ykk::RunClass>(),
                           e->d_sweep_runs.as<ykk::SweepRun>(), e->run_classes, e->d_run_units.as<int>(), e->run_units, bitmap, e->row_words,
                           e->row_stride, pin_on, e->d_class_count.as<int>(), n_long, rstage);
        return YKPRED_OK;
      };
      switch (nit) {
        case 1: TRY(launch_runs(ykk::k_class_runs<1>)); break;
        case 2: TRY(launch_runs(ykk::k_class_runs<2>)); break;
        case 3: TRY(launch_runs(ykk::k_class_runs<3>)); break;
        case 4: TRY(launch_runs(ykk::k_class_runs<4>)); break;
        case 5: TRY(launch_runs(ykk::k_class_runs<5>)); break;
        case 6: TRY(launch_runs(ykk::k_class_runs<6>)); break;
        default: TRY(launch_runs(ykk::k_class_runs<7>)); break;
      }
      tm.end(sz, "k_class_runs");
    }
    if (sweep_rows_on) {
      const int its = (e->row_stride + ykk::kWave - 1) / ykk::kWave;
      int segs = (its + ykk::kWalkMaxIt - 1) / ykk::kWalkMaxIt, nit = (its + segs - 1) / segs;
      while (nit > 1 && ykk::sweep_lds_bytes(nit) > (size_t)e->max_lds_bytes) {
        ++segs;
        nit = (its + segs - 1) / segs;
      }
      const int n_long = segs - (nit * segs - its);
      tm.begin(sz);
      for (int b = 0; b < e->n_big; ++b) {
        const int n_rows = e->sweep_rows[b];
        if (n_rows == 0) continue;
        const int n_units = e->sweep_units[b];
        const int groups = std::max(1, std::min(e->sweep_groups > 0 ? e->sweep_groups : e->num_cus, (n_units + ykk::kSweepWaves - 1) / ykk::kSweepWaves));
        auto launch_sweep = [&](auto kernel) -> int {
          const size_t lds = ykk::sweep_lds_bytes(nit);
          if (lds > 64 * 1024) HIPCHK(hipFuncSetAttribute((const void*)kernel, hipFuncAttributeMaxDynamicSharedMemorySize, (int)lds));
          hipLaunchKernelGGL(kernel, dim3((unsigned)groups, (unsigned)segs), dim3(ykk::kSweepThreads), lds, sz, pc,
                             e->d_ent_c.as<unsigned>() + (size_t)b * 65 * (size_t)e->row_words, e->d_rbits_c.as<u64>() + (size_t)b * ykk::kRankBits * (size_t)e->row_words,
                             e->d_sweep_rows.as<ykk::SweepRow>() + e->sweep_row_off[b], e->d_sweep_runs.as<ykk::SweepRun>(), n_rows,
                             e->d_sweep_units.as<int>() + e->sweep_unit_off[b], n_units, bitmap, e->row_words, e->row_stride, pin_on,
                             e->d_class_count.as<int>(), n_long);
          return YKPRED_OK;
        };
        switch (nit) {
          case 1: TRY(launch_sweep(ykk::k_sweep_rows<1>)); break;
          case 2: TRY(launch_sweep(ykk::k_sweep_rows<2>)); break;
          case 3: TRY(launch_sweep(ykk::k_sweep_rows<3>)); break;
          case 4: TRY(launch_sweep(ykk::k_sweep_rows<4>)); break;
          case 5: TRY(launch_sweep(ykk::k_sweep_rows<5>)); break;
          case 6: TRY(launch_sweep(ykk::k_sweep_rows<6>)); break;
          default: TRY(launch_sweep(ykk::k_sweep_rows<7>)); break;
        }
      }
      tm.end(sz, "k_sweep_rows");
    }
    if (fuse_on) {
      const int wpl = e->fuse_wpl >= 5 ? 5 : (e->fuse_wpl >= 2 ? 2 : (e->fuse_wpl == 1 ? 1 : (e->row_words > 384 ? 5 : (e->row_words > 192 ? 2 : 1))));
      const int gw = ykk::kFuseComputeWaves * ykk::kWave * wpl;
      const unsigned ygroups = (unsigned)((e->row_words + gw - 1) / gw);
      ykk::FuseSrc fsrc{e->planes_canon.as<u64>(), e->fuse_combos > 0 ? e->d_fuse_combo.as<u64>() : nullptr, {e->fam_res.base, e->fam_tol.base, e->fam_aff.base}};
      tm.begin(sz);
      auto launch_fused = [&](auto kernel, const ykk::FuseRec* recs, int n, u64* out, int* counts) {
        hipLaunchKernelGGL(kernel, dim3((unsigned)((n + ykk::kFuseRecsPerBlock - 1) / ykk::kFuseRecsPerBlock), ygroups), dim3(ykk::kBlock), 0, sz, recs, n, fsrc,
                           e->row_words, e->row_stride, out, counts);
      };
      auto launch_wide = [&](const ykk::FuseRec* recs, int n, u64* out, int* counts) {
        if (wpl == 5) launch_fused(ykk::k_fused_rows<5, 8>, recs, n, out, counts);
        else if (wpl == 2) launch_fused(ykk::k_fused_rows<2, 8>, recs, n, out, counts);
        else launch_fused(ykk::k_fused_rows<1, 8>, recs, n, out, counts);
      };
      if (e->fuse_combos > 0) {
        launch_wide(e->d_fuse_combo_rec.as<ykk::FuseRec>(), e->fuse_combos, e->d_fuse_combo.as<u64>(), nullptr);
        if (wpl == 5) launch_fused(ykk::k_fused_rows<5, 2>, e->d_fuse_rec.as<ykk::FuseRec>(), e->fuse_count, bitmap, e->d_class_count.as<int>());
        else if (wpl == 2) launch_fused(ykk::k_fused_rows<2, 2>, e->d_fuse_rec.as<ykk::FuseRec>(), e->fuse_count, bitmap, e->d_class_count.as<int>());
        else launch_fused(ykk::k_fused_rows<1, 2>, e->d_fuse_rec.as<ykk::FuseRec>(), e->fuse_count, bitmap, e->d_class_count.as<int>());
      } else {
        launch_wide(e->d_fuse_rec.as<ykk::FuseRec>(), e->fuse_count, bitmap, e->d_class_count.as<int>());
      }
      tm.end(sz, "k_fused_rows");
    }
    tm.begin(sz);
    int walk_nit = 0, walk_segs = 0, walk_long = 0;
    ykk::WalkStage wstage{};
    wstage.n = (int)e->h_stage_rows.size();
    for (int k = 0; k < wstage.n; ++k) wstage.row[k] = e->h_stage_rows[(size_t)k];
    bool slices = small_chunks && e->combine_slices != 0 && pc.n_big > 0 && pc.res != nullptr && !(use_sweep && e->sweep_min_run <= 1 && listed);
    if (slices) {
      const int its = (e->row_stride + ykk::kWave - 1) / ykk::kWave;
      const size_t lds_cap = std::min((size_t)e->max_lds_bytes, (size_t)80 * 1024);
      walk_segs = (its + ykk::kWalkMaxIt - 1) / ykk::kWalkMaxIt;
      walk_nit = (its + walk_segs - 1) / walk_segs;
      while (walk_nit > 1 && ykk::walk_lds_bytes(pc.n_big, wstage.n, walk_nit) > lds_cap) {
        ++walk_segs;
        walk_nit = (its + walk_segs - 1) / walk_segs;
      }
      walk_long = walk_segs - (walk_nit * walk_segs - its);
      slices = ykk::walk_lds_bytes(pc.n_big, wstage.n, walk_nit) <= (size_t)e->max_lds_bytes && its * ykk::kWave <= e->idx_stride;
    }
    if (slices) {
      HIPCHK(e->d_slice_desc.ensure((size_t)std::max(e->NC, 1) * sizeof(ykk::SliceDesc)));
      HIPCHK(e->d_slice_general.ensure(sizeof(int)));
      HIPCHK(hipMemsetAsync(e->d_slice_general.p, 0, sizeof(int), sz));
      hipLaunchKernelGGL(ykk::k_slice_desc, dim3((unsigned)((e->NC + ykk::kBlock - 1) / ykk::kBlock)), dim3(ykk::kBlock), 0, sz, ct, pc, e->NC, class_dirty,
                         pin_on, e->d_slice_desc.as<ykk::SliceDesc>(), e->d_slice_general.as<int>(), wstage);
      tm.end(sz, "k_slice_desc");
      tm.begin(sz);
      const int per_group = ykk::kRowsWaves * ykk::kWalkChunksPerWave;
      const unsigned gx = (unsigned)((e->NC + per_group - 1) / per_group);
      auto launch_walk = [&](auto kernel, int nit, int segs, int w_base) -> int {
        const size_t lds = ykk::walk_lds_bytes(pc.n_big, wstage.n, nit);
        if (lds > 64 * 1024) HIPCHK(hipFuncSetAttribute((const void*)kernel, hipFuncAttributeMaxDynamicSharedMemorySize, (int)lds));
        hipLaunchKernelGGL(kernel, dim3(gx, (unsigned)segs), dim3(ykk::kRowsThreads), lds, sz, pc, e->d_slice_desc.as<ykk::SliceDesc>(), bitmap,
                           e->row_words, e->row_stride, pin_on, e->d_class_count.as<int>(), e->NC, w_base, wstage);
        return YKPRED_OK;
      };
      auto launch_segments = [&](int nit, int segs, int w_base, bool tail) -> int {
        if (segs <= 0) return YKPRED_OK;
        switch (nit * 2 + (tail ? 1 : 0)) {
#define YK_WALK_CASE(N)                                                         \
  case (N) * 2: return launch_walk(ykk::k_walk_rows<(N), false>, nit, segs, w_base); \
  case (N) * 2 + 1: return launch_walk(ykk::k_walk_rows<(N), true>, nit, segs, w_base);
          YK_WALK_CASE(1) YK_WALK_CASE(2) YK_WALK_CASE(3) YK_WALK_CASE(4) YK_WALK_CASE(5) YK_WALK_CASE(6) YK_WALK_CASE(7)
#undef YK_WALK_CASE
        }
        return fail(e, YKPRED_E_INVALID, "k_walk_rows: no kernel for " + std::to_string(nit) + " word groups per lane");
      };
      {
        const int n_short = walk_segs - walk_long, nit_last = n_short > 0 ? walk_nit - 1 : walk_nit;
        const int long_plain = n_short > 0 ? walk_long : walk_long - 1, short_plain = n_short > 0 ? n_short - 1 : 0;
        TRY(launch_segments(walk_nit, long_plain, 0, false));
        TRY(launch_segments(walk_nit - 1, short_plain, walk_long * walk_nit * ykk::kWave, false));
        TRY(launch_segments(nit_last, 1, (long_plain * walk_nit + short_plain * (walk_nit - 1)) * ykk::kWave, true));
      }
      tm.end(sz, "k_walk_rows");
      tm.begin(sz);
      hipLaunchKernelGGL(ykk::k_combine_wave, dim3((unsigned)((e->NC + ykk::kWavesPerBlock - 1) / ykk::kWavesPerBlock)), dim3(ykk::kBlock), 0, sz, ct,
                         pc, bitmap, e->row_words, e->row_stride, pin_on, e->d_class_count.as<int>(), e->NC, class_dirty,
                         e->d_slice_desc.as<ykk::SliceDesc>(), e->d_slice_general.as<int>(), (const int*)nullptr);
    } else if (counts_early) {
      const ykk::FixRows fix{e->d_class_rows_a.as<u64>(), e->d_fix_row.as<int>(), e->d_fix_slot.as<int>(), e->n_fix_rows};
      const int blocks = n_run + e->n_fix_rows;
      if (blocks > 0)
        hipLaunchKernelGGL(ykk::k_combine, dim3((unsigned)blocks, grid.y), dim3(ykk::kBlock), (size_t)e->combine_lds_bytes, sz, ct, pc, bitmap, e->row_words,
                           e->row_stride, pin_on, (int*)nullptr, tpg, class_dirty, chunk_list, fix, n_run);
    } else if (n_run == 0) {
    } else if (small_chunks) {
      const dim3 wgrid((unsigned)((std::max(n_run, 1) + ykk::kWavesPerBlock - 1) / ykk::kWavesPerBlock));
      hipLaunchKernelGGL(ykk::k_combine_wave, wgrid, dim3(ykk::kBlock), 0, sz, ct, pc, bitmap, e->row_words, e->row_stride, pin_on,
                         e->d_class_count.as<int>(), n_run, class_dirty, (const ykk::SliceDesc*)nullptr, (const int*)nullptr, chunk_list);
    } else {
      hipLaunchKernelGGL(ykk::k_combine, grid, dim3(ykk::kBlock), (size_t)e->combine_lds_bytes, sz, ct, pc, bitmap, e->row_words, e->row_stride,
                         pin_on, e->d_class_count.as<int>(), tpg, class_dirty, chunk_list, ykk::FixRows{nullptr, nullptr, nullptr, 0}, n_run);
    }
    tm.end(sz, dirty_only ? "k_combine(dirty classes)" : "k_combine");
  }
  if (want_dec) {
    HIPCHK(hipEventRecord(e->ev_join, sb));
    HIPCHK(hipStreamWaitEvent(st, e->ev_join, 0));
  }
  if ((want_dec || want_cnt) && !scattered) {
    tm.begin(st);
    hipLaunchKernelGGL(ykk::k_scatter, dim3((unsigned)((P + ykk::kBlock - 1) / ykk::kBlock)), dim3(ykk::kBlock), 0, st, P,
                       e->d_pod_class.as<int>(), e->d_class_count.as<int>(), e->d_class_best.as<int>(), e->d_key.as<u64>(),
                       want_cnt ? (int*)e->last_counts : nullptr, want_dec ? (int*)e->last_decisions : nullptr,
                       want_keys ? (i64*)e->last_keys : nullptr);
    tm.end(st, "k_scatter");
  }
  HIPCHK(hipGetLastError());
  return YKPRED_OK;
  };
  const bool graphable = !tm.on && !e->graph_disabled && !(e->comm && e->comm_world > 1) && !(a->options & (YKPRED_EVAL_DIRECT | YKPRED_EVAL_SPREAD_COUNT_ONLY));
  hipGraphExec_t exec = nullptr;
  if (graphable) {
    ykpred_engine::GraphKey key{e->tables_version, pre, filt, a->options, (void*)bitmap, e->last_counts, e->last_decisions, e->last_keys};
    for (size_t i = 0; i < e->graphs.size();) {
      if (e->graphs[i].first.version != e->tables_version) {
        (void)hipGraphExecDestroy(e->graphs[i].second);
        e->graphs.erase(e->graphs.begin() + (long)i);
      } else {
        if (e->graphs[i].first == key) exec = e->graphs[i].second;
        ++i;
      }
    }
    bool repeated = false;
    for (size_t i = 0; i < e->seen.size();) {
      if (e->seen[i].version != e->tables_version) {
        e->seen.erase(e->seen.begin() + (long)i);
        continue;
      }
      repeated = repeated || e->seen[i] == key;
      ++i;
    }
    if (!repeated && e->seen.size() < 8) e->seen.push_back(key);
    if (!exec && repeated) {
      hipGraph_t g = nullptr;
      int crc = YKPRED_E_DEVICE;
      if (hipStreamBeginCapture(st, hipStreamCaptureModeThreadLocal) == hipSuccess) {
        crc = enqueue();
        if (hipStreamEndCapture(st, &g) != hipSuccess) crc = YKPRED_E_DEVICE;
      }
      if (crc == YKPRED_OK && g && hipGraphInstantiate(&exec, g, nullptr, nullptr, 0) == hipSuccess) {
        if (e->graphs.size() >= 8) {
          (void)hipGraphExecDestroy(e->graphs.front().second);
          e->graphs.erase(e->graphs.begin());
        }
        e->graphs.emplace_back(key, exec);
      } else {
        exec = nullptr;
        e->graph_disabled = true;
        (void)hipGetLastError();
      }
      if (g) (void)hipGraphDestroy(g);
    }
  }
  if (exec) {
    HIPCHK(hipGraphLaunch(exec, st));
  } else {
    int rc = enqueue();
    if (rc < 0) return rc;
    if (rc == 1) {
      tm.done(st);
      return YKPRED_OK;
    }
  }
  tm.done(st);
  if (e->ev_eval_done) (void)hipEventRecord(e->ev_eval_done, st);
  e->bitmap_epoch = e->nodes_epoch;
  e->last_pre = pre;
  e->last_filt = filt;
  e->last_eval_valid = true;
  if (!(a->options & (YKPRED_EVAL_SKIP_BITMAP | YKPRED_EVAL_DIRTY_CLASSES))) e->n_full_evals++;
  if (!(a->options & (YKPRED_EVAL_SKIP_BITMAP | YKPRED_EVAL_DIRTY_CLASSES))) std::fill(e->h_row_stale.begin(), e->h_row_stale.end(), 0);
  if (want_dec) {
    e->win_partial = use_run_decide_pass;
    e->rank_valid = true;
    e->ranked_specs_version = e->specs_version;
    e->ranked_nodes_epoch = e->nodes_epoch;
// ... 2796 lines not shown
  return YKPRED_OK;
}

int32_t ykpred_set_row_capacity(ykpred_engine_t* e, int32_t rows) {
  YK_SERIALISE(e);
  if (!e || rows < 0) return fail(e, YKPRED_E_INVALID, "set_row_capacity: bad argument");
  if (rows && e->rows_total > rows) return fail(e, YKPRED_E_INVALID, "set_row_capacity: the bitmap already uses more rows");
  if (rows != e->row_capacity) e->last_eval_valid = false;
  e->row_capacity = rows;
  e->ask_epoch++;
  return YKPRED_OK;
}

int32_t ykpred_set_row_stride(ykpred_engine_t* e, int32_t words) {
  YK_SERIALISE(e);
  if (!e || words < 0 || words % 16 != 0) return fail(e, YKPRED_E_INVALID, "set_row_stride: need a multiple of 16 words (0 = automatic)");
  e->forced_stride = words;
  e->ask_epoch++;
  return YKPRED_OK;
}

int32_t ykpred_gather_bitmap(ykpred_engine_t* e, void* gathered, void* stream) {
  YK_SERIALISE(e);
  Range roctx_range("ykpred:gather_bitmap");
  if (e) e->n_gathers++;
  if (!e) return YKPRED_E_INVALID;
  if (!e->comm) return fail(e, YKPRED_E_STATE, "gather_bitmap: no communicator (ykpred_comm_init)");
  if (!e->last_eval_valid || !e->last_bitmap) return fail(e, YKPRED_E_STATE, "gather_bitmap: no current evaluation");
  HIPCHK(hipSetDevice(e->cfg.device));
  hipStream_t st = stream ? (hipStream_t)stream : e->own_stream;
  if (e->comm_world > 1 && e->row_capacity == 0)
    return fail(e, YKPRED_E_STATE, "gather_bitmap: the shards must agree on a row capacity first (ykpred_set_row_capacity)");
  const size_t rows = (size_t)std::max(std::max(e->rows_total, e->row_capacity), 1);
  const size_t words = rows * (size_t)e->row_stride;
  if (!gathered) {
    HIPCHK(e->d_gathered.ensure(words * (size_t)e->comm_world * sizeof(u64)));
    gathered = e->d_gathered.p;
  }
  NCCLCHK(rccl()->AllGather(e->last_bitmap, gathered, words, ncclUint64, e->comm, st));
  HIPCHK(e->d_gathered_map.ensure((size_t)std::max(e->P, 1) * (size_t)e->comm_world * sizeof(int)));
  if (e->P) NCCLCHK(rccl()->AllGather(e->d_pod_row.p, e->d_gathered_map.p, (size_t)e->P, ncclInt32, e->comm, st));
  return YKPRED_OK;
}

namespace {
uint64_t layout_digest(ykpred_engine_t* e) {
  if (e->layout_hashed_version == e->layout_version) return e->layout_hash_value;
  uint64_t h = 1469598103934665603ull;
  auto mix = [&](uint64_t v) {
    h ^= v;
    h *= 1099511628211ull;
  };
  mix((uint64_t)e->C);
  mix((uint64_t)e->P);
  mix((uint64_t)e->row_stride);
  mix((uint64_t)std::max(e->rows_total, e->row_capacity));
  mix((uint64_t)e->rows_a);
  for (int p = 0; p < e->P; ++p) mix(((uint64_t)(uint32_t)e->h_pod_row[(size_t)p] << 32) | (uint32_t)e->h_pod_class[(size_t)p]);
  e->layout_hash_value = h;
  e->layout_hashed_version = e->layout_version;
  return h;
}
int expand_class_rows_into(ykpred_engine_t* e, const u64* class_rows, u64* out, hipStream_t st) {
  const int C = e->C, P = e->P;
  if (C == 0 || P == 0) return YKPRED_OK;
  if (e->ident_classes < C) {
    HIPCHK(e->d_class_sig_ident.ensure((size_t)C * 4 * sizeof(int)));
    hipLaunchKernelGGL(ykk::k_identity_sigs, dim3((unsigned)((C + ykk::kBlock - 1) / ykk::kBlock)), dim3(ykk::kBlock), 0, st, C, e->d_class_sig_ident.as<int>());
    e->ident_classes = C;
  }
  HIPCHK(e->d_expand_count.ensure((size_t)C * sizeof(int)));
  ykk::ClassTable ct{e->d_class_sig_ident.as<int>(), e->d_class_pin.as<int>(), e->d_chunk_class.as<int>(), e->d_chunk_begin.as<int>(),
                     e->d_chunk_len.as<int>(), e->d_chunk_first.as<int>(), e->d_members.as<int>(), e->d_chunk_zone.as<int>(), 0, nullptr};
  ykk::Planes pl{nullptr, class_rows, nullptr, nullptr, e->row_stride, nullptr, 0, nullptr, 0, nullptr, 0, nullptr, 0, 0, 0, 0, 0, nullptr, nullptr, nullptr, nullptr, nullptr};
  if (e->n_classes_a > 0) {
    HIPCHK(e->d_class_rows_slot.ensure((size_t)e->n_classes_a * (size_t)e->row_stride * sizeof(u64)));
    hipLaunchKernelGGL(ykk::k_pick_class_rows, dim3((unsigned)e->n_classes_a), dim3(ykk::kBlock), 0, st, class_rows, e->d_class_list_a.as<int>(),
                       e->n_classes_a, e->row_stride, e->d_class_rows_slot.as<u64>());
    const size_t lds_bytes = (size_t)2 * ykk::kBandClasses * (size_t)e->row_stride * sizeof(u64);
    if (lds_bytes > 64 * 1024)
      HIPCHK(hipFuncSetAttribute((const void*)ykk::k_expand_bands, hipFuncAttributeMaxDynamicSharedMemorySize, (int)lds_bytes));
    hipLaunchKernelGGL(ykk::k_expand_bands, dim3((unsigned)ykk::kBandGroups), dim3(ykk::kBandBlock), lds_bytes, st, out, e->d_class_rows_slot.as<u64>(),
                       e->d_band_tab.as<ykk::BandEntry>(), e->n_bands, e->row_stride);
    if (e->n_fix_rows > 0)
      hipLaunchKernelGGL(ykk::k_fix_rows, dim3((unsigned)e->n_fix_rows), dim3(ykk::kBlock), 0, st, out, e->d_class_rows_slot.as<u64>(),
                         e->d_fix_row.as<int>(), e->d_fix_slot.as<int>(), e->n_fix_rows, e->row_stride);
  }
  if ((long)e->NC * e->wave_combine_below > (long)P) {
    hipLaunchKernelGGL(ykk::k_combine_wave, dim3((unsigned)((e->NC + ykk::kWavesPerBlock - 1) / ykk::kWavesPerBlock)), dim3(ykk::kBlock), 0, st, ct, pl,
                       out, e->row_stride, e->row_stride, 0, e->d_expand_count.as<int>(), e->NC, (const int*)nullptr, (const ykk::SliceDesc*)nullptr,
                       (const int*)nullptr, (const int*)nullptr);
  } else {
    int tpg = ykk::kBlock;
    while (tpg > ykk::kWave && (tpg / 2) * 2 >= e->row_stride) tpg /= 2;
    const int seg = tpg * ykk::kCombineUnroll * 2;
    dim3 grid((unsigned)e->NC, (unsigned)((e->row_stride + seg - 1) / seg));
    hipLaunchKernelGGL(ykk::k_combine, grid, dim3(ykk::kBlock), (size_t)e->combine_lds_bytes, st, ct, pl, out, e->row_stride, e->row_stride, 0,
                       e->d_expand_count.as<int>(), tpg, (const int*)nullptr, (const int*)nullptr, ykk::FixRows{nullptr, nullptr, nullptr, 0}, e->NC);
  }
  HIPCHK(hipGetLastError());
  return YKPRED_OK;
}
int expand_peer_rows_into(ykpred_engine_t* e, const u64* class_rows, const int* pod_class, u64* out, hipStream_t st) {
  if (e->P == 0) return YKPRED_OK;
  const int n_rows = std::max(std::max(e->rows_total, e->row_capacity), 1);
  if (e->row_pod_version != e->layout_version) {
    HIPCHK(e->d_row_pod.ensure((size_t)n_rows * sizeof(int)));
    HIPCHK(hipMemsetAsync(e->d_row_pod.p, 0xff, (size_t)n_rows * sizeof(int), st));
    hipLaunchKernelGGL(ykk::k_invert_row_map, dim3((unsigned)((e->P + ykk::kBlock - 1) / ykk::kBlock)), dim3(ykk::kBlock), 0, st, e->d_pod_row.as<int>(), e->P,
                       e->d_row_pod.as<int>());
    e->row_pod_version = e->layout_version;
  }
  const int row_groups = (n_rows + ykk::kExpandRows - 1) / ykk::kExpandRows;
  hipLaunchKernelGGL(ykk::k_expand_by_row, dim3((unsigned)((row_groups + ykk::kWavesPerBlock - 1) / ykk::kWavesPerBlock)), dim3(ykk::kBlock), 0, st, out, class_rows,
                     pod_class, e->d_row_pod.as<int>(), n_rows, e->row_stride);
  HIPCHK(hipGetLastError());
  return YKPRED_OK;
}
int collect_class_rows_into(ykpred_engine_t* e, u64* out, hipStream_t st) {
  if (e->C == 0) return YKPRED_OK;
  hipLaunchKernelGGL(ykk::k_collect_class_rows, dim3((unsigned)e->C), dim3(ykk::kBlock), 0, st, (const u64*)e->last_bitmap, e->C,
                     e->d_class_first.as<int>(), e->d_pod_row.as<int>(), e->row_stride, out);
  HIPCHK(hipGetLastError());
  return YKPRED_OK;
}
}

int32_t ykpred_layout_hash(ykpred_engine_t* e, uint64_t* out) {
  YK_SERIALISE(e);
  if (!e || !out) return fail(e, YKPRED_E_INVALID, "layout_hash: null argument");
  if (e->classes_dirty || (int)e->h_pod_row.size() < e->P) return fail(e, YKPRED_E_STATE, "layout_hash: no current class build (run ykpred_eval)");
  *out = layout_digest(e);
  return YKPRED_OK;
}

int32_t ykpred_collect_class_rows(ykpred_engine_t* e, void* out, void* stream) {
  YK_SERIALISE(e);
  if (!e || !out) return fail(e, YKPRED_E_INVALID, "collect_class_rows: null argument");
  if (e->classes_dirty || !e->last_eval_valid || !e->last_bitmap) return fail(e, YKPRED_E_STATE, "collect_class_rows: no current evaluation");
  HIPCHK(hipSetDevice(e->cfg.device));
  return collect_class_rows_into(e, (u64*)out, stream ? (hipStream_t)stream : e->own_stream);
}

int32_t ykpred_read_class_rows(ykpred_engine_t* e, uint64_t* out) {
  YK_SERIALISE(e);
  if (!e || !out) return fail(e, YKPRED_E_INVALID, "read_class_rows: null argument");
  if (e->classes_dirty || !e->last_eval_valid || !e->last_bitmap) return fail(e, YKPRED_E_STATE, "read_class_rows: no current evaluation");
  if (e->C == 0 || e->row_words == 0) return YKPRED_OK;
  HIPCHK(hipSetDevice(e->cfg.device));
  hipStream_t st = e->peek_stream ? e->peek_stream : e->own_stream;
  if (e->ev_eval_done) HIPCHK(hipStreamWaitEvent(st, e->ev_eval_done, 0));
  const size_t bytes = (size_t)e->C * (size_t)e->row_stride * sizeof(u64);
  HIPCHK(e->d_class_rows_all.ensure(bytes));
  TRY(collect_class_rows_into(e, e->d_class_rows_all.as<u64>(), st));
  HIPCHK(hipMemcpy2DAsync(out, (size_t)e->row_words * sizeof(u64), e->d_class_rows_all.p, (size_t)e->row_stride * sizeof(u64), (size_t)e->row_words * sizeof(u64),
                          (size_t)e->C, hipMemcpyDeviceToHost, st));
  HIPCHK(hipStreamSynchronize(st));
  return YKPRED_OK;
}

int32_t ykpred_expand_class_rows(ykpred_engine_t* e, const void* class_rows, const int32_t* pod_class, void* bitmap_out, void* stream) {
  YK_SERIALISE(e);
  if (!e || !class_rows || !bitmap_out) return fail(e, YKPRED_E_INVALID, "expand_class_rows: null argument");
  if (e->classes_dirty) return fail(e, YKPRED_E_STATE, "expand_class_rows: no current class build (run ykpred_eval)");
  HIPCHK(hipSetDevice(e->cfg.device));
  hipStream_t st = stream ? (hipStream_t)stream : e->own_stream;
  if (!pod_class) return expand_class_rows_into(e, (const u64*)class_rows, (u64*)bitmap_out, st);
  return expand_peer_rows_into(e, (const u64*)class_rows, (const int*)pod_class, (u64*)bitmap_out, st);
}

int32_t ykpred_gather_bitmap_compressed(ykpred_engine_t* e, void* gathered, void* stream) {
  YK_SERIALISE(e);
  Range roctx_range("ykpred:gather_bitmap_compressed");
  if (e) e->n_gathers++;
  if (!e) return YKPRED_E_INVALID;
  if (!e->comm) return fail(e, YKPRED_E_STATE, "gather_bitmap_compressed: no communicator (ykpred_comm_init)");
  if (e->classes_dirty || !e->last_eval_valid || !e->last_bitmap) return fail(e, YKPRED_E_STATE, "gather_bitmap_compressed: no current evaluation");
  HIPCHK(hipSetDevice(e->cfg.device));
  hipStream_t st = stream ? (hipStream_t)stream : e->own_stream;
  const int G = e->comm_world;
  if (G > 1 && e->row_capacity == 0)
// ... 110 lines not shown
```

yunikorn-k8shim_amd/csrc/engine/kernels.hip.h:

```cpp
#pragma once
#include <hip/hip_runtime.h>
#include <stdint.h>

#include <type_traits>

namespace ykk {

typedef unsigned long long u64;
typedef long long i64;

constexpr int kMaxR = 8;
constexpr int kMaxKT = 4;
constexpr int kMaxW = 8;
constexpr int kMaxWTotal = 32;
constexpr int kMaxKD = 8;
constexpr int kMaxKP = 4;

constexpr int kWave = 64;
constexpr int kBlock = 256;
constexpr int kWavesPerBlock = kBlock / kWave;
constexpr int kSigsPerBlock = 16;
constexpr int kSigsPerBlockMany = 64;
constexpr int kManySigs = 4096;
__host__ __device__ inline int sigs_per_block(int D) { return D > kManySigs ? kSigsPerBlockMany : kSigsPerBlock; }
// ... 487 lines not shown
      if (b == lane) keep = m;
    }
    u64* dst = is_label ? o.req + (size_t)(c * 64 + lane) * o.stride
                        : (is_taint ? o.taint + (size_t)((c - t.W) * 64 + lane) * o.stride
                                    : o.port + (size_t)((c - t.W - t.KT) * 64 + lane) * o.stride);
    dst[word] = keep;
  } else {
    u64 un = __ballot(n >= 0 && (t.flags[n >= 0 ? n : 0] & kNodeUnschedulable));
    u64 ex = __ballot(n >= 0);
    if (lane == 0) {
      o.unsched[word] = un;
      o.exists[word] = ex;
    }
  }
}

__global__ __launch_bounds__(kBlock) void k_base_planes(NodeTable t, const int* __restrict__ perm, BasePlanes o, int n_words) {
  if ((int)blockIdx.x < t.W + t.KT + t.KP + 1) plane_base(t, perm, o, n_words);
}

struct SigPlaneArgs {
  BasePlanes base;
  PlaneOut tol, aff;
  const u64* sig_tol;
  const unsigned* sig_tolflags;
  const u64* sig_ports;
  int KP;
  u64 taint_used[kMaxKT];
  AffSigs affs;
  int KT, W;
  unsigned pre_mask, filt_mask;
  int n_words;
};
constexpr int kBitSigsPerBlock = 8;

template <int WPL>
__device__ __forceinline__ void dnf_words(const u64* __restrict__ terms, int t0, int t1, int W, const u64* __restrict__ req, int stride,
                                          const int (&w)[WPL], u64 (&any)[WPL]) {
#pragma unroll
  for (int j = 0; j < WPL; ++j) any[j] = 0;
  for (int t = t0; t < t1; ++t) {
    u64 all[WPL];
#pragma unroll
    for (int j = 0; j < WPL; ++j) all[j] = ~0ull;
    for (int k = 0; k < W; ++k) {
      u64 m = terms[(size_t)t * W + k];
      while (m) {
        int q = __ffsll((long long)m) - 1;
        m &= m - 1;
        const u64* row = req + (size_t)(k * 64 + q) * stride;
#pragma unroll
        for (int j = 0; j < WPL; ++j) all[j] &= row[w[j]];
      }
    }
#pragma unroll
    for (int j = 0; j < WPL; ++j) any[j] |= all[j];
  }
}
constexpr int kSigTermRegs = 4;
template <int WPL>
__device__ __forceinline__ void dnf_words_regs(const u64 (&tw)[kSigTermRegs], int j0, int j1, int W, const u64* __restrict__ req, int stride,
                                               const int (&w)[WPL], u64 (&any)[WPL]) {
#pragma unroll
  for (int j = 0; j < WPL; ++j) any[j] = 0;
  for (int jj = j0; jj < j1;) {
    u64 all[WPL];
#pragma unroll
    for (int j = 0; j < WPL; ++j) all[j] = ~0ull;
    for (int k = 0; k < W; ++k, ++jj) {
      const int r = jj >> 6, l = jj & 63;
      u64 m = (u64)readlane_i64((i64)(r == 0 ? tw[0] : (r == 1 ? tw[1] : (r == 2 ? tw[2] : tw[3]))), l);
      while (m) {
        int q = __ffsll((long long)m) - 1;
        m &= m - 1;
        const u64* row = req + (size_t)(k * 64 + q) * stride;
#pragma unroll
        for (int j = 0; j < WPL; ++j) all[j] &= row[w[j]];
      }
    }
#pragma unroll
    for (int j = 0; j < WPL; ++j) any[j] |= all[j];
  }
}
template <int WPL>
__global__ __launch_bounds__(kBlock) void k_sig_planes(SigPlaneArgs a) {
  const int lane = threadIdx.x % kWave;
  const int wbase = (blockIdx.y * kWavesPerBlock + threadIdx.x / kWave) * (kWave * WPL);
  if (wbase >= a.n_words) return;
  int w[WPL], w_raw[WPL];
  bool live[WPL];
  u64 exists[WPL];
#pragma unroll
  for (int j = 0; j < WPL; ++j) {
    w_raw[j] = wbase + j * kWave + lane;
    live[j] = w_raw[j] < a.n_words;
    w[j] = live[j] ? w_raw[j] : a.n_words - 1;
    exists[j] = a.base.exists[w[j]];
  }
  auto note_first = [&](int* first, int d, const u64 (&val)[WPL]) {
    if (!first) return;
    int fw = kNoWord;
#pragma unroll
    for (int j = WPL - 1; j >= 0; --j) {
      const u64 nz = __ballot(live[j] && val[j] != 0);
      if (nz) fw = wbase + j * kWave + __ffsll((long long)nz) - 1;
    }
    if (fw != kNoWord && lane == 0) atomicMin(&first[d], fw);
  };
  const int d0 = blockIdx.x * kBitSigsPerBlock;
  if (blockIdx.z == 0) {
    const int nd = min(kBitSigsPerBlock, a.tol.D - d0);
    if (nd <= 0) return;
    const bool taint_en = a.filt_mask & kPlugTaint, unsched_en = a.filt_mask & kPlugUnsched;
    const bool ports_en = (a.filt_mask & kPlugPorts) && (a.pre_mask & kPlugPorts);
    u64 unsched[WPL];
#pragma unroll
    for (int j = 0; j < WPL; ++j) unsched[j] = unsched_en ? a.base.unsched[w[j]] : 0ull;
    const bool batch = nd * a.KT <= kWave && nd * a.KP <= kWave;
    const unsigned fl_l = lane < nd ? a.sig_tolflags[d0 + lane] : 0u;
    u64 tol_l = 0, port_l = 0;
    if (batch) {
      if (lane < nd * a.KT) tol_l = a.sig_tol[(size_t)d0 * a.KT + lane];
      if (ports_en && lane < nd * a.KP) port_l = a.sig_ports[(size_t)d0 * a.KP + lane];
    }
    for (int i = 0; i < nd; ++i) {
      const int d = d0 + i;
      const unsigned fl = (unsigned)__builtin_amdgcn_readlane((int)fl_l, i);
      u64 bad[WPL];
#pragma unroll
      for (int j = 0; j < WPL; ++j) bad[j] = 0;
      if (taint_en)
        for (int k = 0; k < a.KT; ++k) {
          const u64 tolerated = batch ? (u64)readlane_i64((i64)tol_l, i * a.KT + k) : a.sig_tol[(size_t)d * a.KT + k];
          u64 m = ~tolerated & a.taint_used[k];
          while (m) {
            int tt = __ffsll((long long)m) - 1;
            m &= m - 1;
            const u64* row = a.base.taint + (size_t)(k * 64 + tt) * a.base.stride;
#pragma unroll
            for (int j = 0; j < WPL; ++j) bad[j] |= row[w[j]];
          }
        }
      if (ports_en)
        for (int k = 0; k < a.KP; ++k) {
          u64 m = batch ? (u64)readlane_i64((i64)port_l, i * a.KP + k) : a.sig_ports[(size_t)d * a.KP + k];
          while (m) {
            int pp = __ffsll((long long)m) - 1;
            m &= m - 1;
            const u64* row = a.base.port + (size_t)(k * 64 + pp) * a.base.stride;
#pragma unroll
            for (int j = 0; j < WPL; ++j) bad[j] |= row[w[j]];
          }
        }
      u64 val[WPL];
#pragma unroll
      for (int j = 0; j < WPL; ++j) {
        u64 b = bad[j];
        if (!(fl & kSpecToleratesUnsched)) b |= unsched[j];
        if (fl & kSpecUnsupported) b = ~0ull;
        val[j] = exists[j] & ~b;
        if (live[j]) a.tol.canon[(size_t)d * a.tol.stride + w[j]] = val[j];
      }
      note_first(a.tol.first, d, val);
    }
  } else {
    const int nd = min(kBitSigsPerBlock, a.aff.D - d0);
    if (nd <= 0) return;
    const bool pre_en = a.pre_mask & kPlugAffinity, filt_en = a.filt_mask & kPlugAffinity;
    const unsigned f_l = lane < nd ? a.affs.flags[d0 + lane] : 0u;
    const int to_l = lane <= nd ? a.affs.term_off[d0 + lane] : 0;
    const int tbase = __builtin_amdgcn_readlane(to_l, 0);
    const int n_mask_words = (__builtin_amdgcn_readlane(to_l, nd) - tbase) * a.W;
    const bool batch = filt_en && n_mask_words <= kSigTermRegs * kWave;
    u64 tw[kSigTermRegs];
#pragma unroll
    for (int r = 0; r < kSigTermRegs; ++r) {
      const int j = r * kWave + lane;
      tw[r] = batch && j < n_mask_words ? a.affs.terms[(size_t)tbase * a.W + j] : 0ull;
    }
    for (int i = 0; i < nd; ++i) {
      const int d = d0 + i;
      const unsigned f = (unsigned)__builtin_amdgcn_readlane((int)f_l, i);
      const bool skip = pre_en && (f & kSpecAffSkip);
      u64 ok[WPL];
#pragma unroll
      for (int j = 0; j < WPL; ++j) ok[j] = exists[j];
      if (pre_en && !skip) {
        if (f & kSpecPreReject) {
#pragma unroll
          for (int j = 0; j < WPL; ++j) ok[j] = 0;
        }
        if (f & kSpecPreNames) {
          u64 any[WPL];
          dnf_words<WPL>(a.affs.pre_terms, a.affs.pre_off[d], a.affs.pre_off[d + 1], a.W, a.base.req, a.base.stride, w, any);
#pragma unroll
          for (int j = 0; j < WPL; ++j) ok[j] &= any[j];
        }
      }
      if (filt_en && !skip) {
        const int t0 = __builtin_amdgcn_readlane(to_l, i), t1 = __builtin_amdgcn_readlane(to_l, i + 1);
        u64 any[WPL];
        if (batch)
          dnf_words_regs<WPL>(tw, (t0 - tbase) * a.W, (t1 - tbase) * a.W, a.W, a.base.req, a.base.stride, w, any);
        else
          dnf_words<WPL>(a.affs.terms, t0, t1, a.W, a.base.req, a.base.stride, w, any);
#pragma unroll
        for (int j = 0; j < WPL; ++j) ok[j] &= any[j];
      }
#pragma unroll
      for (int j = 0; j < WPL; ++j)
        if (live[j]) a.aff.canon[(size_t)d * a.aff.stride + w[j]] = ok[j];
      note_first(a.aff.first, d, ok);
    }
  }
}

__global__ __launch_bounds__(kBlock) void k_permute_planes(int n_nodes, const int* __restrict__ perm, const u64* __restrict__ canon,
                                                           u64* __restrict__ ranked, int stride, int n_rows, int n_words,
                                                           int* __restrict__ first ) {
  const int wave = threadIdx.x / kWave, lane = threadIdx.x % kWave;
  const int w = blockIdx.y * kWavesPerBlock + wave;
  if (w >= n_words) return;
  const int pos = w * kWave + lane;
  const int src = pos < n_nodes ? perm[pos] : -1;
  const int sw = src >> 6, sb = src & 63;
  const int spb = sigs_per_block(n_rows);
  const int d0 = blockIdx.x * spb;
  const int dend = min(d0 + spb, n_rows);
  u64 keep = 0;
  for (int d = d0; d < dend; ++d) {
    bool bit = src >= 0 && ((canon[(size_t)d * stride + sw] >> sb) & 1ull);
    u64 b = __ballot(bit);
    if (d - d0 == lane) keep = b;
  }
  if (lane < dend - d0) {
    ranked[(size_t)(d0 + lane) * stride + w] = keep;
    if (first && keep) atomicMin(&first[d0 + lane], w);
  }
}

struct SpreadC {
  int kd, ks, max_skew, min_domains, self_match;
  unsigned flags;
  int cnt_off, dom_size;
  int kind;
};
struct SpreadSigs {
  int D;
  const int* c_off;
// ... 254 lines not shown
  }
  auto add = [&](const u64* p, int global_row) {
#pragma unroll
    for (int i = 0; i < kMaxClassRows; ++i)
      if (i == cr.n) cr.row[i] = p;
    ++cr.n;
    if (pl.first) cr.start = max(cr.start, pl.first[global_row]);
  };
  if (pl.tol && st >= 0) add(pl.tol + (size_t)st * pl.stride, pl.base_tol + st);
  if (pl.aff && sa >= 0) add(pl.aff + (size_t)sa * pl.stride, pl.base_aff + sa);
  if (pl.spread && ss >= 0) add(pl.spread + (size_t)ss * pl.stride, pl.base_spread + ss);
  if (pl.res && sr >= 0) {
    const int* rr = pl.res_rows + (size_t)sr * pl.res_slots;
    for (int k = 0; k < pl.res_slots; ++k) {
      const int r = rr[k];
      if (r < 0) continue;
      const int big = r >> kRowBigShift, rid = r & ((1 << kRowBigShift) - 1);
      if (big) {
        int first_word = -1;
        if (pl.pfx) {
          const i64 v = pl.res_val[rid];
          const i64* px = pl.pfx + (size_t)(big - 1) * pl.n_words;
          int lo = 0, hi = pl.n_words;
          while (lo < hi) {
            const int mid = (lo + hi) >> 1;
            if (px[mid] < v) lo = mid + 1; else hi = mid;
          }
          first_word = lo < pl.n_words ? lo : kNoWord;
          if (pl.first) cr.start = max(cr.start, first_word);
        }
#pragma unroll
        for (int i = 0; i < kMaxIdxRows; ++i)
          if (i == cr.ni) {
            cr.ipm[i] = pl.pmask + (size_t)(big - 1) * pl.n_words * 65;
            if (pl.res_win) {
              cr.irow[i] = pl.res_win + (size_t)rid * 64;
              cr.isf[i] = pl.sfree + (size_t)(big - 1) * pl.n_words * 64;
              cr.ival[i] = pl.res_val[rid];
              cr.ig4[i] = (first_word >= 0 && first_word != kNoWord) ? (first_word >> 2) : 0x3fffffff;
            } else {
              cr.irow[i] = pl.res_idx + (size_t)rid * pl.idx_stride;
            }
          }
        ++cr.ni;
      } else {
        add(pl.res + (size_t)rid * pl.stride, pl.base_res + rid);
      }
    }
  }
  return cr;
}
__device__ __forceinline__ u64 class_idx_word(const ClassRows& cr, int w) {
  u64 v = ~0ull;
#pragma unroll
  for (int i = 0; i < kMaxIdxRows; ++i)
    if (i < cr.ni) {
      int pos;
      if (!cr.isf[i]) {
        pos = cr.irow[i][w];
      } else if ((unsigned)((w >> 2) - cr.ig4[i]) < 16u) {
        pos = cr.irow[i][w & 63];
      } else {
        const i64* sf = cr.isf[i] + (size_t)w * 64;
        int lo = 0, hi = 64;
        while (lo < hi) {
          const int mid = (lo + hi) >> 1;
          if (sf[mid] < cr.ival[i]) lo = mid + 1; else hi = mid;
        }
        pos = lo;
      }
      v &= cr.ipm[i][(size_t)w * 65 + min(pos, 64)];
    }
  return v;
}
__device__ __forceinline__ u64 class_word(const ClassRows& cr, int w) {
  u64 v = ~0ull;
#pragma unroll
  for (int i = 0; i < kMaxClassRows; ++i)
    if (i < cr.n) v &= cr.row[i][w];
  if (cr.ni) v &= class_idx_word(cr, w);
  return v;
}

struct FixRows {
  const u64* class_rows;
  const int* rows;
  const int* slots;
  int n;
};
__device__ __forceinline__ void fix_row(const FixRows& f, int i, u64* __restrict__ out, int row_stride) {
  typedef u64 u64x2 __attribute__((ext_vector_type(2)));
  if (i >= f.n) return;
  const u64* src = f.class_rows + (size_t)f.slots[i] * row_stride;
  u64* dst = out + (size_t)f.rows[i] * row_stride;
  for (int w = threadIdx.x * 2; w < row_stride; w += 2 * kBlock) *(u64x2*)(dst + w) = *(const u64x2*)(src + w);
}
__global__ __launch_bounds__(kBlock) void k_combine(ClassTable ct, Planes pl, u64* __restrict__ bitmap, int row_words, int row_stride,
                                                    int pin_enabled, int* __restrict__ class_count, int tpg,
                                                    const int* __restrict__ class_dirty ,
                                                    const int* __restrict__ chunk_list ,
                                                    FixRows fix ,
                                                    int n_run) {
  constexpr int WPL = 2;
  if ((int)blockIdx.x >= n_run) {
    if (blockIdx.y == 0) fix_row(fix, (int)blockIdx.x - n_run, bitmap, row_stride);
    return;
  }
  const bool all_fail = pin_enabled & 2;
  pin_enabled &= 1;
  const int chunk = chunk_list ? chunk_list[blockIdx.x] : (int)blockIdx.x;
  const int cls = ct.chunk_class[chunk];
  if (class_dirty ? !class_dirty[cls] : chunk_elsewhere(ct, chunk)) return;
  const int begin = ct.chunk_begin[chunk];
  const int len = ct.chunk_len[chunk];
  const int sr = ct.sig[cls * 4 + 0], st = ct.sig[cls * 4 + 1], sa = ct.sig[cls * 4 + 2], ss = ct.sig[cls * 4 + 3];
  const int pin = pin_enabled ? ct.pin[cls] : -1;
  const int lane = threadIdx.x % kWave;
  const int group = threadIdx.x / tpg, groups = kBlock / tpg, t = threadIdx.x % tpg;
  const int seg_base = blockIdx.y * (tpg * kCombineUnroll * WPL);
  const ClassRows cr = class_rows(pl, sr, st, sa, ss);

  u64 v[kCombineUnroll][WPL];
  int pc = 0;
#pragma unroll
  for (int u = 0; u < kCombineUnroll; ++u) {
#pragma unroll
    for (int j = 0; j < WPL; ++j) {
      int w = seg_base + (u * tpg + t) * WPL + j;
      u64 x = 0;
      if (w < row_words) {
        x = class_word(cr, w);
        if (pin == -2 || all_fail)
          x = 0;
        else if (pin >= 0)
          x &= (w == (pin >> 6)) ? (1ull << (pin & 63)) : 0ull;
      }
      v[u][j] = x;
      pc += __popcll(x);
    }
  }
  if (ct.chunk_first[chunk] && group == 0) {
#pragma unroll
    for (int off = 32; off > 0; off >>= 1) pc += __shfl_down(pc, off, kWave);
    if (lane == 0 && pc && class_count) atomicAdd(&class_count[cls], pc);
  }
  int mine = lane < len ? ct.members[begin + lane] : 0;
  for (int i = group; i < len; i += groups) {
    int p = __builtin_amdgcn_readlane(mine, i);
    if (p < 0) continue;
    u64* row = bitmap + (size_t)p * row_stride;
#pragma unroll
    for (int u = 0; u < kCombineUnroll; ++u) {
      int w = seg_base + (u * tpg + t) * WPL;
      if (w < row_stride) {
        typedef u64 u64x2 __attribute__((ext_vector_type(2)));
        *(u64x2*)(row + w) = u64x2{v[u][0], v[u][1]};
      }
    }
  }
}

struct SliceDesc;
__device__ __forceinline__ bool slice_desc_general(const SliceDesc* desc, int chunk);
__global__ __launch_bounds__(kBlock) __attribute__((amdgpu_waves_per_eu(5, 8))) void k_combine_wave(ClassTable ct, Planes pl, u64* __restrict__ bitmap, int row_words, int row_stride,
                                                         int pin_enabled, int* __restrict__ class_count, int n_chunks,
                                                         const int* __restrict__ class_dirty ,
                                                         const SliceDesc* __restrict__ only_general ,
                                                         const int* __restrict__ n_general ,
                                                         const int* __restrict__ chunk_list ) {
  typedef u64 u64x2 __attribute__((ext_vector_type(2)));
  const bool all_fail = pin_enabled & 2;
  pin_enabled &= 1;
  const int slot = blockIdx.x * kWavesPerBlock + threadIdx.x / kWave;
  if (slot >= n_chunks) return;
  const int chunk = chunk_list ? chunk_list[slot] : slot;
  if (only_general && (*n_general == 0 || !slice_desc_general(only_general, chunk))) return;
  const int lane = threadIdx.x % kWave;
  const int cls = ct.chunk_class[chunk];
  if (class_dirty ? !class_dirty[cls] : chunk_elsewhere(ct, chunk)) return;
  const int begin = ct.chunk_begin[chunk], len = ct.chunk_len[chunk];
  const int sr = ct.sig[cls * 4 + 0], st = ct.sig[cls * 4 + 1], sa = ct.sig[cls * 4 + 2], ss = ct.sig[cls * 4 + 3];
  const int pin = pin_enabled ? ct.pin[cls] : -1;
  const ClassRows cr = class_rows(pl, sr, st, sa, ss);
  const int mine = lane < len ? ct.members[begin + lane] : -1;
  int pc = 0;
  auto class_pair = [&](int w) {
    u64x2 x = {0, 0};
    if (w < row_words && pin != -2 && !all_fail) {
      x = u64x2{~0ull, ~0ull};
#pragma unroll
// ... 628 lines not shown
    u64 base[NIT];
    {
      const ConstRun* cr = (const ConstRun*)(unsigned long long)(runs + run);
      const int st = cr->st, sa = cr->sa, ss = cr->ss;
      const u64* p0 = pl.res + w_first + lane;
      const u64* pt = (pl.tol && st >= 0) ? pl.tol + (size_t)st * pl.stride + w_first + lane : p0;
      const u64* pa = (pl.aff && sa >= 0) ? pl.aff + (size_t)sa * pl.stride + w_first + lane : p0;
      const u64* ps = (pl.spread && ss >= 0) ? pl.spread + (size_t)ss * pl.stride + w_first + lane : p0;
#pragma unroll
      for (int it = 0; it < NIT; ++it) {
        const u64 v = p0[it * kWave] & pt[it * kWave] & pa[it * kWave] & ps[it * kWave];
        base[it] = (w_first + it * kWave + lane < rw && it < nit) ? v : 0ull;
      }
    }
    for (;;) {
      const int cls = __builtin_amdgcn_readfirstlane(da.x), dest0 = __builtin_amdgcn_readfirstlane(da.y);
      const int len = __builtin_amdgcn_readfirstlane(da.z), slots = __builtin_amdgcn_readfirstlane(da.w);
      u64 m[NIT];
      int cnt = 0;
      {
        const u64* r0 = s_stage + (slots & 255) * SW + lane;
        const u64* r1 = s_stage + ((slots >> 8) & 255) * SW + lane;
        const u64* r2 = s_stage + ((slots >> 16) & 255) * SW + lane;
        const u64* r3 = s_stage + ((slots >> 24) & 255) * SW + lane;
#pragma unroll
        for (int it = 0; it < NIT; ++it) {
          m[it] = base[it] & r0[it * kWave] & r1[it * kWave] & r2[it * kWave] & r3[it * kWave];
          cnt += __popcll(m[it]);
        }
      }
      const int pc = __builtin_amdgcn_readlane(wave_sum_lane63(cnt), 63);
      ++c;
      bool more = true;
      if (c == c1) {
        if (c < unit_end) {
          cb = c;
          if (lane < 2 * kRunsBatch) s_desc[lane] = d_nx;
          c1 = min(cb + kRunsBatch, unit_end);
          d_nx = fetch(c1);
        } else {
          u += unit_step;
          if (u >= n_units) {
            more = false;
          } else {
            cb = ub[u], unit_end = ub[u + 1];
            d_nx = fetch(cb);
            if (lane < 2 * kRunsBatch) s_desc[lane] = d_nx;
            c = cb;
            c1 = min(cb + kRunsBatch, unit_end);
            d_nx = fetch(c1);
          }
        }
      }
      if (more) da = s_desc[2 * (c - cb)], db = s_desc[2 * (c - cb) + 1];
      u64* dst = bitmap + (size_t)dest0 * row_stride + w_first + lane;
      for (int i = 0; i < len; ++i, dst += row_stride) {
#pragma unroll
        for (int it = 0; it < NIT; ++it) {
          if (it < NIT - 2) {
            dst[it * kWave] = m[it];
          } else if (it < nit) {
            if (!last_seg || it < nit - 1 || w_first + it * kWave + lane < row_stride) dst[it * kWave] = m[it];
          }
        }
      }
      if (lane == 63 && pc) atomicAdd(&class_count[cls], pc);
      if (!more) return;
      if (__builtin_amdgcn_readfirstlane(db.x) != run) break;
    }
  }
}

constexpr int kBandGroups = 256;
constexpr int kBandClasses = 4;
constexpr int kBandMaxLds = 150 * 1024;
struct BandEntry {
  int slot[kBandClasses];
  int xb[kBandClasses - 1];
  int sb[kBandClasses - 1];
  int steps, first_step;
  int n, pad;
};

__global__ __launch_bounds__(kBlock) void k_class_rows(ClassTable ct, Planes pl, const int* __restrict__ class_list, int n_list, int row_words,
                                                       int row_stride, int pin_enabled, u64* __restrict__ row_table,
                                                       int* __restrict__ class_count, const int* __restrict__ class_dirty,
                                                       const int* __restrict__ class_list_b, int n_b) {
  typedef u64 u64x2 __attribute__((ext_vector_type(2)));
  const bool all_fail = pin_enabled & 2;
  pin_enabled &= 1;
  const int k = blockIdx.x * kWavesPerBlock + threadIdx.x / kWave;
  if (k >= n_list + n_b) return;
  const bool store = k < n_list;
  const int cls = store ? class_list[k] : class_list_b[k - n_list];
  if (class_dirty && !class_dirty[cls]) return;
  const int lane = threadIdx.x % kWave;
  const int sr = ct.sig[cls * 4 + 0], st = ct.sig[cls * 4 + 1], sa = ct.sig[cls * 4 + 2], ss = ct.sig[cls * 4 + 3];
  const int pin = pin_enabled ? ct.pin[cls] : -1;
  const ClassRows cr = class_rows(pl, sr, st, sa, ss);
  u64* dst = row_table + (size_t)k * row_stride;
  int pc = 0;
  for (int w = 2 * lane; w < row_stride; w += 2 * kWave) {
    u64x2 x = {0, 0};
    if (w < row_words && pin != -2 && !all_fail) {
      x = u64x2{~0ull, ~0ull};
#pragma unroll
      for (int i = 0; i < kMaxClassRows; ++i)
        if (i < cr.n) x &= *(const u64x2*)(cr.row[i] + w);
      if (cr.ni) {
        x.x &= class_idx_word(cr, w);
        if (w + 1 < row_words) x.y &= class_idx_word(cr, w + 1);
      }
      if (w + 1 >= row_words) x.y = 0;
      if (pin >= 0) {
        x.x &= (w == (pin >> 6)) ? (1ull << (pin & 63)) : 0ull;
        x.y &= (w + 1 == (pin >> 6)) ? (1ull << (pin & 63)) : 0ull;
      }
    }
    pc += __popcll(x.x) + __popcll(x.y);
    if (store) *(u64x2*)(dst + w) = x;
  }
#pragma unroll
  for (int off = 32; off > 0; off >>= 1) pc += __shfl_down(pc, off, kWave);
  if (lane == 0) class_count[cls] = pc;
}

constexpr int kBandBlock = kBlock + kWave;
__global__ __launch_bounds__(kBandBlock) void k_expand_bands(u64* __restrict__ out, const u64* __restrict__ class_rows,
                                                             const BandEntry* __restrict__ tab, int n_bands, int row_stride) {
  typedef u64 u64x2 __attribute__((ext_vector_type(2)));
  extern __shared__ u64 band_lds[];
  const int b = blockIdx.x, tid = threadIdx.x;
  const int row_b = row_stride * 8;
  constexpr long kWin = (long)kBandGroups * 4096;
  if (tid >= kBlock) {
    const int lane = tid - kBlock;
    const int pieces = row_stride / 2;
    auto load_rows = [&](int band) {
      const BandEntry be = tab[(size_t)band * kBandGroups + b];
#pragma unroll
      for (int c = 0; c < kBandClasses; ++c) {
        if (c >= be.n && c > 0) break;
        const u64x2* src = (const u64x2*)(class_rows + (size_t)be.slot[c] * row_stride);
        u64x2* dst = (u64x2*)(band_lds + (size_t)((band & 1) * kBandClasses + c) * row_stride);
        for (int i0 = 0; i0 < pieces; i0 += 4 * kWave) {
          u64x2 r[4];
#pragma unroll
          for (int k = 0; k < 4; ++k)
            if (i0 + k * kWave + lane < pieces) r[k] = src[i0 + k * kWave + lane];
#pragma unroll
          for (int k = 0; k < 4; ++k)
            if (i0 + k * kWave + lane < pieces) dst[i0 + k * kWave + lane] = r[k];
        }
      }
    };
    load_rows(0);
    __syncthreads();
    for (int band = 0; band < n_bands; ++band) {
      if (band + 1 < n_bands) load_rows(band + 1);
      __syncthreads();
    }
    return;
  }
  __syncthreads();
  const int p = b * 4096 + tid * 16;
  const unsigned urow_b = (unsigned)row_b;
  const unsigned dcol = (unsigned)(kWin % row_b);
  unsigned ucol = (unsigned)(p % row_b);
  for (int band = 0; band < n_bands; ++band) {
    const BandEntry cur = tab[(size_t)band * kBandGroups + b];
    const int s0 = cur.first_step, s1 = s0 + cur.steps;
    const char* lds = (const char*)(band_lds + (size_t)(band & 1) * kBandClasses * row_stride);
    unsigned kb[kBandClasses - 1];
#pragma unroll
    for (int i = 0; i < kBandClasses - 1; ++i)
      kb[i] = cur.xb[i] == 0x7fffffff ? 0xffffffffu : (((unsigned)cur.xb[i] << 8) | (unsigned)(cur.sb[i] - s0));
    char* win_base = (char*)out + (long)s0 * kWin;
    auto run_band = [&](auto ncls_tag) {
      constexpr int kN = decltype(ncls_tag)::value;
      constexpr int kU = 4;
      for (int s = s0; s < s1; s += kU) {
        u64x2 v[kU];
        bool live[kU];
#pragma unroll
        for (int u = 0; u < kU; ++u) {
          unsigned off = ucol;
          live[u] = p >= (int)ucol;
          if (kN > 1) {
            const unsigned key = ((unsigned)(p - (int)ucol) << 8) | (unsigned)(s + u - s0);
#pragma unroll
            for (int i = 0; i < kN - 1; ++i) off += key >= kb[i] ? urow_b : 0u;
          }
          v[u] = *(const u64x2*)(lds + off);
          const unsigned t = ucol + dcol;
          ucol = min(t, t - urow_b);
        }
#pragma unroll
        for (int u = 0; u < kU; ++u) {
          if (live[u]) *(u64x2*)(win_base + p) = v[u];
          win_base += kWin;
        }
      }
    };
    if (cur.n <= 1)
      run_band(std::integral_constant<int, 1>{});
    else if (cur.n == 2)
      run_band(std::integral_constant<int, 2>{});
    else if (cur.n == 3)
      run_band(std::integral_constant<int, 3>{});
    else
      run_band(std::integral_constant<int, kBandClasses>{});
    __syncthreads();
  }
}
__global__ __launch_bounds__(kBlock) void k_fix_rows(u64* __restrict__ out, const u64* __restrict__ class_rows, const int* __restrict__ rows,
                                                     const int* __restrict__ slots, int n, int row_stride) {
  typedef u64 u64x2 __attribute__((ext_vector_type(2)));
  if ((int)blockIdx.x >= n) return;
  const u64* src = class_rows + (size_t)slots[blockIdx.x] * row_stride;
  u64* dst = out + (size_t)rows[blockIdx.x] * row_stride;
  for (int w = threadIdx.x * 2; w < row_stride; w += 2 * kBlock) *(u64x2*)(dst + w) = *(const u64x2*)(src + w);
}

__global__ __launch_bounds__(kBlock) void k_decide(ClassTable ct, Planes ranked, int n_classes, int row_words, const int* __restrict__ perm,
                                                   const int* __restrict__ rank, int pin_enabled, int* __restrict__ class_best, int eager) {
  int cls = blockIdx.x * kWavesPerBlock + threadIdx.x / kWave;
  if (cls >= n_classes) return;
  if (ct.decide_list) cls = ct.decide_list[cls];
  const int lane = threadIdx.x % kWave;
  const int sr = ct.sig[cls * 4 + 0], st = ct.sig[cls * 4 + 1], sa = ct.sig[cls * 4 + 2], ss = ct.sig[cls * 4 + 3];
  const bool all_fail = pin_enabled & 2;
  const int pin = (pin_enabled & 1) ? ct.pin[cls] : -1;
  int best = -1;
  const ClassRows cr = class_rows(ranked, sr, st, sa, ss);
  if (pin == -2 || all_fail) {
    best = -1;
  } else if (pin >= 0) {
    int pos = rank[pin];
    u64 x = class_word(cr, pos >> 6);
    best = ((x >> (pos & 63)) & 1ull) ? pin : -1;
  } else {
    for (int base = cr.start & ~(kWave - 1); base < row_words; base += kWave) {
      int w = base + lane;
      u64 x = w < row_words ? ~0ull : 0ull;
      if (eager) {
        const int ws = w < row_words ? w : 0;
        u64 y = ~0ull;
#pragma unroll
        for (int i = 0; i < kMaxClassRows; ++i)
          if (i < cr.n) y &= cr.row[i][ws];
        if (cr.ni) y &= class_idx_word(cr, ws);
        x &= y;
      } else {
        if (cr.ni && x) x &= class_idx_word(cr, w);
#pragma unroll
        for (int i = kMaxClassRows - 1; i >= 0; --i)
          if (i < cr.n && x) x &= cr.row[i][w];
      }
      u64 any = __ballot(x != 0);
      if (any) {
        int first_lane = __ffsll((long long)any) - 1;
        u64 xw = __shfl(x, first_lane, kWave);
        int pos = (base + first_lane) * kWave + (__ffsll((long long)xw) - 1);
        best = perm[pos];
        break;
      }
    }
  }
  if (lane == 0) class_best[cls] = best;
}

constexpr int kDecideGroups = 4, kDecideLanes = kWave / kDecideGroups;
__global__ __launch_bounds__(kBlock) void k_decide_groups(ClassTable ct, Planes ranked, int n_classes, int row_words, const int* __restrict__ perm,
                                                          const int* __restrict__ rank, int pin_enabled, int* __restrict__ class_best) {
  const int wave = blockIdx.x * kWavesPerBlock + threadIdx.x / kWave;
  const int lane = threadIdx.x % kWave, g = lane / kDecideLanes, l = lane % kDecideLanes;
  const int cls_raw = wave * kDecideGroups + g;
  const bool live = cls_raw < n_classes;
  const int cls = ct.decide_list ? ct.decide_list[live ? cls_raw : n_classes - 1] : (live ? cls_raw : n_classes - 1);
  const bool all_fail = pin_enabled & 2;
  const int sr = ct.sig[cls * 4 + 0], st = ct.sig[cls * 4 + 1], sa = ct.sig[cls * 4 + 2], ss = ct.sig[cls * 4 + 3];
  const int pin = (pin_enabled & 1) ? ct.pin[cls] : -1;
  const ClassRows cr = class_rows(ranked, sr, st, sa, ss);
  auto word_at = [&](int w) {
    u64 x = w < row_words ? ~0ull : 0ull;
    if (cr.ni && x) x &= class_idx_word(cr, w);
#pragma unroll
    for (int i = kMaxClassRows - 1; i >= 0; --i)
      if (i < cr.n && x) x &= cr.row[i][w];
    return x;
  };
  int best = -1;
  bool done = !live || pin == -2 || all_fail;
  if (!done && pin >= 0) {
    const int pos = rank[pin];
    const u64 x = word_at(pos >> 6);
    best = ((x >> (pos & 63)) & 1ull) ? pin : -1;
    done = true;
  }
  const int w0 = cr.start >= row_words ? row_words : (cr.start & ~(kDecideLanes - 1));
  for (int t = 0;; ++t) {
    const int base = w0 + t * kDecideLanes;
    if (base >= row_words) done = true;
    if (__ballot(!done) == 0) break;
// ... 2938 lines not shown
```

Baseline: 40340 billion evals/s.

## Fuse zone-B row writes into k_class_rows, drop fix-rows, widen sig planes

Band packing now skips rows that straddle a band window, so the separate fix-row copy kernel and its fused path in k_combine can be removed. When zone-B bitmap rows are small (under a configurable KB threshold) and counts are computed early, k_class_rows writes those rows directly in 16-row groups, and the k_combine launch is skipped. The signature-plane kernel gains a signatures-per-block template parameter and drops to narrower blocks when the grid would be too small to fill the CUs. The costs are some wasted bitmap row slots at window edges and repeated recomputation of each class's AND row for every 16-row group.

```diff
diff --git a/yunikorn-k8shim_amd/csrc/engine/engine.hip b/yunikorn-k8shim_amd/csrc/engine/engine.hip
--- a/yunikorn-k8shim_amd/csrc/engine/engine.hip
+++ b/yunikorn-k8shim_amd/csrc/engine/engine.hip
@@ -311,9 +311,11 @@
   int round_node_assume = 1;
   int round_prof = 0;
   int fail_after = 0;
+  int sig_wide = -1;
   int sig_wpl = 0;
   int combine_slices = 1;
   int decide_groups_from = 16384;
+  int head_zone_b_kb = 16384;
   int early_counts = 1;
   int group_lds = -1;
   int group_scratch_mb = 256;
@@ -321,11 +323,13 @@
   int group_chunk_tasks = 0;
   int max_lds_bytes = 64 * 1024;
   int num_cus = 256;
-  int n_bands = 0, n_band_steps = 0, n_classes_a = 0, n_fix_rows = 0;
+  int n_bands = 0, n_band_steps = 0, n_classes_a = 0;
   std::vector<int32_t> h_class_slot_a;
-  DevBuf d_band_tab, d_class_rows_a, d_class_list_a, d_class_slot_a, d_fix_row, d_fix_slot, d_chunk_zone;
+  DevBuf d_band_tab, d_class_rows_a, d_class_list_a, d_class_slot_a, d_chunk_zone;
   DevBuf d_class_list_b;
   int n_classes_b = 0;
+  DevBuf d_groups_b;
+  int n_groups_b = 0;
   std::vector<int32_t> h_ch_zone;
   std::vector<uint8_t> h_row_stale;
   std::vector<int32_t> h_class_sig, h_class_pin, h_class_first, h_class_live;
@@ -538,6 +542,7 @@
   }
   const long row_b = (long)e->row_stride * 8, win = (long)ykk::kBandGroups * 4096;
   const int KC = ykk::kBandClasses;
+  const long win_rows = win % row_b == 0 ? win / row_b : win / row_b - 1;
   auto piece_min_of = [&](int steps) { return (int)((double)steps * (4096.0 + (double)row_b) / (double)row_b / (double)(KC - 1) * 1.3) + 3; };
   int S = e->band_steps;
   if (S <= 0) {
@@ -560,7 +565,7 @@
   e->h_class_slot_a.assign((size_t)C, -1);
   e->h_pod_row.assign((size_t)P, -1);
   std::vector<ykk::BandEntry> band_tab;
-  std::vector<int32_t> class_list_a, fix_row, fix_slot;
+  std::vector<int32_t> class_list_a;
   int n_steps = 0, n_bands = 0, rows_a = 0;
   const bool geometry_ok = e->bands_enabled && e->N > 0 && (size_t)2 * KC * (size_t)row_b <= (size_t)std::min(ykk::kBandMaxLds, e->max_lds_bytes);
   if (geometry_ok) {
@@ -571,7 +576,7 @@
         class_list_a.push_back(c);
         rows_needed += class_size[(size_t)c];
       }
-    if (rows_needed < (long)S * win / row_b / 4) {
+    if (rows_needed < (long)S * win_rows / 4) {
       class_list_a.clear();
       std::fill(e->h_class_slot_a.begin(), e->h_class_slot_a.end(), -1);
     }
@@ -587,21 +592,22 @@
     std::vector<Piece> pieces;
     int band = 0;
     while (ci < class_list_a.size() && ok) {
-      const long band_rows = (long)S * win / row_b;
+      const long band_rows = (long)S * win_rows;
       long remaining = left;
       for (size_t k = ci + 1; k < class_list_a.size() && remaining <= band_rows; ++k) remaining += class_size[(size_t)class_list_a[k]];
       const long s_lo = (long)band * S;
       long band_steps_now = S;
       if (remaining + piece_min + 2 < band_rows) {
-        band_steps_now = ((remaining + piece_min + 2) * row_b + win - 1) / win;
+        band_steps_now = (remaining + piece_min + 2 + win_rows - 1) / win_rows;
         band_steps_now = std::min<long>(S, std::max<long>(4, (band_steps_now + 3) / 4 * 4));
       }
       const long s_hi = s_lo + band_steps_now;
       const long r_lo = (s_lo * win + row_b - 1) / row_b, r_hi = (s_hi * win + row_b - 1) / row_b;
-      keys.resize((size_t)(r_hi - r_lo));
-      for (size_t i = 0; i < keys.size(); ++i) {
-        const long r = r_lo + (long)i, start = r * row_b;
-        keys[i] = ((uint64_t)(start % win) << 42) | ((uint64_t)(start / win) << 21) | (uint64_t)i;
+      keys.clear();
+      for (long r = r_lo; r < r_hi; ++r) {
+        const long start = r * row_b;
+        if (start % win + row_b > win) continue;
+        keys.push_back(((uint64_t)(start % win) << 42) | ((uint64_t)(start / win) << 21) | (uint64_t)(r - r_lo));
       }
       std::sort(keys.begin(), keys.end());
       pieces.clear();
@@ -675,16 +681,6 @@
       n_steps = n_bands = rows_a = 0;
     } else {
       n_bands = band;
-      std::vector<int32_t> row_slot((size_t)rows_a, -1);
-      for (int c : class_list_a)
-        for (int i = class_off[(size_t)c]; i < class_off[(size_t)c + 1]; ++i) row_slot[(size_t)e->h_pod_row[(size_t)members[(size_t)i]]] = e->h_class_slot_a[(size_t)c];
-      for (long s1 = 1; s1 <= n_steps; ++s1) {
-        const long r = (s1 * win - 1) / row_b;
-        if (r * row_b + row_b > s1 * win && r < rows_a && row_slot[(size_t)r] >= 0) {
-          fix_row.push_back((int32_t)r);
-          fix_slot.push_back(row_slot[(size_t)r]);
-        }
-      }
     }
   }
   int next_row = rows_a;
@@ -811,6 +807,12 @@
     }
     e->n_classes_b = (int)order_b.size();
     TRY(upload(e, e->d_class_list_b, order_b.data(), order_b.size(), st));
+    std::vector<ykk::RowGroup> groups_b;
+    for (int32_t c : order_b)
+      for (int32_t i = 0; i < class_size[(size_t)c]; i += ykk::kRowGroupRows)
+        groups_b.push_back({c, first_row_of[(size_t)c] + i, std::min<int32_t>(ykk::kRowGroupRows, class_size[(size_t)c] - i), i == 0 ? 1 : 0});
+    e->n_groups_b = (int)groups_b.size();
+    TRY(upload(e, e->d_groups_b, groups_b.data(), groups_b.size(), st));
     std::vector<ykk::SweepRun> runs;
     e->run_classes = e->run_units = e->run_rows = 0;
     if (runs_possible) {
@@ -1069,7 +1071,6 @@
   e->n_bands = n_bands;
   e->n_band_steps = n_steps;
   e->n_classes_a = (int)class_list_a.size();
-  e->n_fix_rows = (int)fix_row.size();
   if (e->row_capacity && e->rows_total > e->row_capacity)
     return fail(e, YKPRED_E_INVALID, "the bitmap needs more rows than ykpred_set_row_capacity allows");
   const int cm = e->chunk_members;
@@ -1127,8 +1128,6 @@
   TRY(upload(e, e->d_band_tab, band_tab.data(), band_tab.size(), st));
   TRY(upload(e, e->d_class_list_a, class_list_a.data(), class_list_a.size(), st));
   TRY(upload(e, e->d_class_slot_a, e->h_class_slot_a.data(), e->h_class_slot_a.size(), st));
-  TRY(upload(e, e->d_fix_row, fix_row.data(), fix_row.size(), st));
-  TRY(upload(e, e->d_fix_slot, fix_slot.data(), fix_slot.size(), st));
   HIPCHK(e->d_class_rows_a.ensure((size_t)std::max<size_t>(class_list_a.size(), 1) * (size_t)e->row_stride * sizeof(u64)));
   TRY(upload(e, e->d_chunk_class, ch_class.data(), ch_class.size(), st));
   TRY(upload(e, e->d_chunk_begin, ch_begin.data(), ch_begin.size(), st));
@@ -1548,10 +1547,12 @@
       const int val = eq == std::string::npos ? 1 : atoi(item.c_str() + eq + 1);
       if (key == "walk_rows") e->walk_rows = std::max(val, 1);
       else if (key == "sig_wpl") e->sig_wpl = val;
+      else if (key == "sig_wide") e->sig_wide = val;
       else if (key == "combine_slices") e->combine_slices = val;
       else if (key == "decide_groups_from") e->decide_groups_from = val;
       else if (key == "graph") e->graph_disabled = val != 1;
       else if (key == "early_counts") e->early_counts = val;
+      else if (key == "head_zone_b_kb") e->head_zone_b_kb = std::max(val, 0);
       else if (key == "band_steps") {
         e->bands_enabled = val >= 0;
         e->band_steps = val > 0 ? std::min(256, std::max(4, (val + 3) / 4 * 4)) : 0;
@@ -1624,7 +1625,7 @@
                     &e->d_sfree_r, &e->d_pmask_r, &e->d_rbits_c, &e->d_sorted, &e->d_sorted_off, &e->d_ent_c, &e->d_agree, &e->d_topo_agree, &e->d_bytes_gather, &e->d_fuse_rec, &e->d_fuse_combo_rec, &e->d_fuse_combo, &e->d_run_ranges, &e->d_no_decide, &e->d_glin_r, &e->d_run_classes, &e->d_run_units, &e->d_sweep_rows, &e->d_sweep_runs, &e->d_sweep_units, &e->d_chunk_list_b0, &e->d_walk2_order, &e->d_walk2_big, &e->d_walk2_begin, &e->d_walk2_len, &e->d_idx_c, &e->d_win_r, &e->d_pfx_r, &e->d_slice_desc, &e->d_slice_general, &e->d_chunk_list_b, &e->d_first_r, &e->d_sig_tol, &e->d_sig_tolflags, &e->d_sig_aff_flags, &e->d_sig_aff_off,
                     &e->d_sig_aff_terms, &e->d_sig_pre_off, &e->d_sig_pre_terms, &e->d_pod_spec, &e->d_pod_pin, &e->d_pod_class,
                     &e->d_class_sig, &e->d_class_pin, &e->d_class_first, &e->d_class_word, &e->d_chunk_class, &e->d_chunk_begin, &e->d_chunk_len, &e->d_chunk_first,
-                    &e->d_pod_row, &e->d_band_tab, &e->d_class_rows_a, &e->d_class_list_a, &e->d_class_slot_a, &e->d_fix_row, &e->d_fix_slot, &e->d_chunk_zone,
+                    &e->d_pod_row, &e->d_band_tab, &e->d_class_rows_a, &e->d_class_list_a, &e->d_class_slot_a, &e->d_chunk_zone,
                     &e->d_members, &e->d_patches, &e->d_rows, &e->d_row_count, &e->d_row_best, &e->d_class_count, &e->d_class_best, &e->d_bitmap, &e->d_counts, &e->d_decisions, &e->d_keys, &e->d_scratch,
                     &e->d_member_key, &e->d_name_rank, &e->d_member_tie, &e->d_class_rows_all, &e->d_gathered_classes, &e->d_class_rows_slot,
                     &e->d_class_sig_ident, &e->d_expand_count, &e->d_layout_hash, &e->d_gathered_pod_class, &e->d_row_pod,
@@ -2314,15 +2315,27 @@
     sa.filt_mask = filt;
     sa.n_words = e->row_words;
     tm.begin(s);
-    const int wpl = e->sig_wpl > 0 ? e->sig_wpl : (e->row_words >= 4 * ykk::kWave ? 4 : (e->row_words >= 2 * ykk::kWave ? 2 : 1));
-    const unsigned chunks = std::max((unsigned)((std::max(sa.tol.D, sa.aff.D) + ykk::kBitSigsPerBlock - 1) / ykk::kBitSigsPerBlock), 1u);
+    int wpl = e->sig_wpl > 0 ? e->sig_wpl : (e->row_words >= 4 * ykk::kWave ? 4 : (e->row_words >= 2 * ykk::kWave ? 2 : 1));
+    int spb = ykk::kBitSigsPerBlock;
+    auto blocks_of = [&](int w, int sp) {
+      return (long)((sa.tol.D + sp - 1) / sp + (sa.aff.D + sp - 1) / sp) * ((e->row_words + ykk::kBlock * w - 1) / (ykk::kBlock * w));
+    };
+    if (e->sig_wide > 0 || (e->sig_wide < 0 && e->sig_wpl <= 0 && blocks_of(wpl, spb) < 2L * e->num_cus)) {
+      wpl = 1;
+      while (spb > 2 && (e->sig_wide > 0 || blocks_of(1, spb) < 2L * e->num_cus)) spb /= 2;
+    }
+    const unsigned chunks = std::max((unsigned)((std::max(sa.tol.D, sa.aff.D) + spb - 1) / spb), 1u);
     const unsigned ygroups = (unsigned)((e->row_words + ykk::kBlock * wpl - 1) / (ykk::kBlock * wpl));
-    if (wpl >= 4)
-      hipLaunchKernelGGL(ykk::k_sig_planes<4>, dim3(chunks, ygroups, 2u), dim3(ykk::kBlock), 0, s, sa);
+    if (spb == 2)
+      hipLaunchKernelGGL((ykk::k_sig_planes<1, 2>), dim3(chunks, ygroups, 2u), dim3(ykk::kBlock), 0, s, sa);
+    else if (spb == 4)
+      hipLaunchKernelGGL((ykk::k_sig_planes<1, 4>), dim3(chunks, ygroups, 2u), dim3(ykk::kBlock), 0, s, sa);
+    else if (wpl >= 4)
+      hipLaunchKernelGGL((ykk::k_sig_planes<4, ykk::kBitSigsPerBlock>), dim3(chunks, ygroups, 2u), dim3(ykk::kBlock), 0, s, sa);
     else if (wpl >= 2)
-      hipLaunchKernelGGL(ykk::k_sig_planes<2>, dim3(chunks, ygroups, 2u), dim3(ykk::kBlock), 0, s, sa);
+      hipLaunchKernelGGL((ykk::k_sig_planes<2, ykk::kBitSigsPerBlock>), dim3(chunks, ygroups, 2u), dim3(ykk::kBlock), 0, s, sa);
     else
-      hipLaunchKernelGGL(ykk::k_sig_planes<1>, dim3(chunks, ygroups, 2u), dim3(ykk::kBlock), 0, s, sa);
+      hipLaunchKernelGGL((ykk::k_sig_planes<1, ykk::kBitSigsPerBlock>), dim3(chunks, ygroups, 2u), dim3(ykk::kBlock), 0, s, sa);
     tm.end(s, sig_name);
     return YKPRED_OK;
   };
@@ -2450,6 +2463,7 @@
   }
   const bool small_chunks = (long)e->NC * e->wave_combine_below > (long)P;
   const bool counts_early = e->early_counts != 0 && !skip_combine && !dirty_only && e->n_classes_a > 0 && e->patch_chunks == 0 && !small_chunks && e->n_classes_b <= 16384;
+  const bool head_zone_b = counts_early && (long)(e->rows_total - e->rows_a) * e->row_stride * 8 <= (long)e->head_zone_b_kb * 1024;
   bool scattered = false;
   if (!skip_combine && !dirty_only && !counts_early) {
     if (zero_counts_beside) HIPCHK(hipStreamWaitEvent(st, e->ev_zero, 0));
@@ -2467,10 +2481,11 @@
     hipStream_t sz = st;
     if (!dirty_only && e->n_classes_a > 0) {
       tm.begin(st);
-      const int n_counted_b = counts_early ? e->n_classes_b : 0;
+      const int n_counted_b = head_zone_b ? e->n_groups_b : (counts_early ? e->n_classes_b : 0);
       hipLaunchKernelGGL(ykk::k_class_rows, dim3((unsigned)((e->n_classes_a + n_counted_b + ykk::kWavesPerBlock - 1) / ykk::kWavesPerBlock)), dim3(ykk::kBlock), 0, st,
                          ct, pc, e->d_class_list_a.as<int>(), e->n_classes_a, e->row_words, e->row_stride, pin_on, e->d_class_rows_a.as<u64>(),
-                         e->d_class_count.as<int>(), (const int*)nullptr, e->d_class_list_b.as<int>(), n_counted_b);
+                         e->d_class_count.as<int>(), (const int*)nullptr, e->d_class_list_b.as<int>(), n_counted_b,
+                         head_zone_b ? e->d_groups_b.as<ykk::RowGroup>() : (const ykk::RowGroup*)nullptr, bitmap);
       tm.end(st, "k_class_rows");
       if (counts_early && want_dec) {
         HIPCHK(hipEventRecord(e->ev_counts, st));
@@ -2488,9 +2503,6 @@
       tm.begin(st);
       hipLaunchKernelGGL(ykk::k_expand_bands, dim3((unsigned)ykk::kBandGroups), dim3(ykk::kBandBlock), lds_bytes, st, bitmap,
                          e->d_class_rows_a.as<u64>(), e->d_band_tab.as<ykk::BandEntry>(), e->n_bands, e->row_stride);
-      if (e->n_fix_rows > 0 && !counts_early)
-        hipLaunchKernelGGL(ykk::k_fix_rows, dim3((unsigned)e->n_fix_rows), dim3(ykk::kBlock), 0, st, bitmap, e->d_class_rows_a.as<u64>(),
-                           e->d_fix_row.as<int>(), e->d_fix_slot.as<int>(), e->n_fix_rows, e->row_stride);
       tm.end(st, "k_expand_bands");
     }
     if (use_sweep && e->run_classes > 0) {
@@ -2645,12 +2657,11 @@
       hipLaunchKernelGGL(ykk::k_combine_wave, dim3((unsigned)((e->NC + ykk::kWavesPerBlock - 1) / ykk::kWavesPerBlock)), dim3(ykk::kBlock), 0, sz, ct,
                          pc, bitmap, e->row_words, e->row_stride, pin_on, e->d_class_count.as<int>(), e->NC, class_dirty,
                          e->d_slice_desc.as<ykk::SliceDesc>(), e->d_slice_general.as<int>(), (const int*)nullptr);
+    } else if (head_zone_b) {
     } else if (counts_early) {
-      const ykk::FixRows fix{e->d_class_rows_a.as<u64>(), e->d_fix_row.as<int>(), e->d_fix_slot.as<int>(), e->n_fix_rows};
-      const int blocks = n_run + e->n_fix_rows;
-      if (blocks > 0)
-        hipLaunchKernelGGL(ykk::k_combine, dim3((unsigned)blocks, grid.y), dim3(ykk::kBlock), (size_t)e->combine_lds_bytes, sz, ct, pc, bitmap, e->row_words,
-                           e->row_stride, pin_on, (int*)nullptr, tpg, class_dirty, chunk_list, fix, n_run);
+      if (n_run > 0)
+        hipLaunchKernelGGL(ykk::k_combine, grid, dim3(ykk::kBlock), (size_t)e->combine_lds_bytes, sz, ct, pc, bitmap, e->row_words,
+                           e->row_stride, pin_on, (int*)nullptr, tpg, class_dirty, chunk_list, n_run);
     } else if (n_run == 0) {
     } else if (small_chunks) {
       const dim3 wgrid((unsigned)((std::max(n_run, 1) + ykk::kWavesPerBlock - 1) / ykk::kWavesPerBlock));
@@ -2658,9 +2669,9 @@
                          e->d_class_count.as<int>(), n_run, class_dirty, (const ykk::SliceDesc*)nullptr, (const int*)nullptr, chunk_list);
     } else {
       hipLaunchKernelGGL(ykk::k_combine, grid, dim3(ykk::kBlock), (size_t)e->combine_lds_bytes, sz, ct, pc, bitmap, e->row_words, e->row_stride,
-                         pin_on, e->d_class_count.as<int>(), tpg, class_dirty, chunk_list, ykk::FixRows{nullptr, nullptr, nullptr, 0}, n_run);
-    }
-    tm.end(sz, dirty_only ? "k_combine(dirty classes)" : "k_combine");
+                         pin_on, e->d_class_count.as<int>(), tpg, class_dirty, chunk_list, n_run);
+    }
+    if (!head_zone_b) tm.end(sz, dirty_only ? "k_combine(dirty classes)" : "k_combine");
   }
   if (want_dec) {
     HIPCHK(hipEventRecord(e->ev_join, sb));
@@ -5623,9 +5634,6 @@
       HIPCHK(hipFuncSetAttribute((const void*)ykk::k_expand_bands, hipFuncAttributeMaxDynamicSharedMemorySize, (int)lds_bytes));
     hipLaunchKernelGGL(ykk::k_expand_bands, dim3((unsigned)ykk::kBandGroups), dim3(ykk::kBandBlock), lds_bytes, st, out, e->d_class_rows_slot.as<u64>(),
                        e->d_band_tab.as<ykk::BandEntry>(), e->n_bands, e->row_stride);
-    if (e->n_fix_rows > 0)
-      hipLaunchKernelGGL(ykk::k_fix_rows, dim3((unsigned)e->n_fix_rows), dim3(ykk::kBlock), 0, st, out, e->d_class_rows_slot.as<u64>(),
-                         e->d_fix_row.as<int>(), e->d_fix_slot.as<int>(), e->n_fix_rows, e->row_stride);
   }
   if ((long)e->NC * e->wave_combine_below > (long)P) {
     hipLaunchKernelGGL(ykk::k_combine_wave, dim3((unsigned)((e->NC + ykk::kWavesPerBlock - 1) / ykk::kWavesPerBlock)), dim3(ykk::kBlock), 0, st, ct, pl,
@@ -5637,7 +5645,7 @@
     const int seg = tpg * ykk::kCombineUnroll * 2;
     dim3 grid((unsigned)e->NC, (unsigned)((e->row_stride + seg - 1) / seg));
     hipLaunchKernelGGL(ykk::k_combine, grid, dim3(ykk::kBlock), (size_t)e->combine_lds_bytes, st, ct, pl, out, e->row_stride, e->row_stride, 0,
-                       e->d_expand_count.as<int>(), tpg, (const int*)nullptr, (const int*)nullptr, ykk::FixRows{nullptr, nullptr, nullptr, 0}, e->NC);
+                       e->d_expand_count.as<int>(), tpg, (const int*)nullptr, (const int*)nullptr, e->NC);
   }
   HIPCHK(hipGetLastError());
   return YKPRED_OK;
diff --git a/yunikorn-k8shim_amd/csrc/engine/kernels.hip.h b/yunikorn-k8shim_amd/csrc/engine/kernels.hip.h
--- a/yunikorn-k8shim_amd/csrc/engine/kernels.hip.h
+++ b/yunikorn-k8shim_amd/csrc/engine/kernels.hip.h
@@ -593,7 +593,7 @@
     for (int j = 0; j < WPL; ++j) any[j] |= all[j];
   }
 }
-template <int WPL>
+template <int WPL, int SPB>
 __global__ __launch_bounds__(kBlock) void k_sig_planes(SigPlaneArgs a) {
   const int lane = threadIdx.x % kWave;
   const int wbase = (blockIdx.y * kWavesPerBlock + threadIdx.x / kWave) * (kWave * WPL);
@@ -618,9 +618,9 @@
     }
     if (fw != kNoWord && lane == 0) atomicMin(&first[d], fw);
   };
-  const int d0 = blockIdx.x * kBitSigsPerBlock;
+  const int d0 = blockIdx.x * SPB;
   if (blockIdx.z == 0) {
-    const int nd = min(kBitSigsPerBlock, a.tol.D - d0);
+    const int nd = min(SPB, a.tol.D - d0);
     if (nd <= 0) return;
     const bool taint_en = a.filt_mask & kPlugTaint, unsched_en = a.filt_mask & kPlugUnsched;
     const bool ports_en = (a.filt_mask & kPlugPorts) && (a.pre_mask & kPlugPorts);
@@ -675,7 +675,7 @@
       note_first(a.tol.first, d, val);
     }
   } else {
-    const int nd = min(kBitSigsPerBlock, a.aff.D - d0);
+    const int nd = min(SPB, a.aff.D - d0);
     if (nd <= 0) return;
     const bool pre_en = a.pre_mask & kPlugAffinity, filt_en = a.filt_mask & kPlugAffinity;
     const unsigned f_l = lane < nd ? a.affs.flags[d0 + lane] : 0u;
@@ -1096,30 +1096,13 @@
   return v;
 }
 
-struct FixRows {
-  const u64* class_rows;
-  const int* rows;
-  const int* slots;
-  int n;
-};
-__device__ __forceinline__ void fix_row(const FixRows& f, int i, u64* __restrict__ out, int row_stride) {
-  typedef u64 u64x2 __attribute__((ext_vector_type(2)));
-  if (i >= f.n) return;
-  const u64* src = f.class_rows + (size_t)f.slots[i] * row_stride;
-  u64* dst = out + (size_t)f.rows[i] * row_stride;
-  for (int w = threadIdx.x * 2; w < row_stride; w += 2 * kBlock) *(u64x2*)(dst + w) = *(const u64x2*)(src + w);
-}
 __global__ __launch_bounds__(kBlock) void k_combine(ClassTable ct, Planes pl, u64* __restrict__ bitmap, int row_words, int row_stride,
                                                     int pin_enabled, int* __restrict__ class_count, int tpg,
                                                     const int* __restrict__ class_dirty ,
                                                     const int* __restrict__ chunk_list ,
-                                                    FixRows fix ,
                                                     int n_run) {
   constexpr int WPL = 2;
-  if ((int)blockIdx.x >= n_run) {
-    if (blockIdx.y == 0) fix_row(fix, (int)blockIdx.x - n_run, bitmap, row_stride);
-    return;
-  }
+  if ((int)blockIdx.x >= n_run) return;
   const bool all_fail = pin_enabled & 2;
   pin_enabled &= 1;
   const int chunk = chunk_list ? chunk_list[blockIdx.x] : (int)blockIdx.x;
@@ -1914,17 +1897,33 @@
   int n, pad;
 };
 
+constexpr int kRowGroupRows = 16;
+struct RowGroup {
+  int cls, first_row, n;
+  int counts;
+};
 __global__ __launch_bounds__(kBlock) void k_class_rows(ClassTable ct, Planes pl, const int* __restrict__ class_list, int n_list, int row_words,
                                                        int row_stride, int pin_enabled, u64* __restrict__ row_table,
                                                        int* __restrict__ class_count, const int* __restrict__ class_dirty,
-                                                       const int* __restrict__ class_list_b, int n_b) {
+                                                       const int* __restrict__ class_list_b, int n_b,
+                                                       const RowGroup* __restrict__ groups_b, u64* __restrict__ bitmap) {
   typedef u64 u64x2 __attribute__((ext_vector_type(2)));
   const bool all_fail = pin_enabled & 2;
   pin_enabled &= 1;
   const int k = blockIdx.x * kWavesPerBlock + threadIdx.x / kWave;
   if (k >= n_list + n_b) return;
   const bool store = k < n_list;
-  const int cls = store ? class_list[k] : class_list_b[k - n_list];
+  int cls, n_rows = 0, counts = 1;
+  u64* rows = nullptr;
+  if (store) {
+    cls = class_list[k];
+  } else if (groups_b) {
+    const RowGroup g = groups_b[k - n_list];
+    cls = g.cls, n_rows = g.n, counts = g.counts;
+    rows = bitmap + (size_t)g.first_row * row_stride;
+  } else {
+    cls = class_list_b[k - n_list];
+  }
   if (class_dirty && !class_dirty[cls]) return;
   const int lane = threadIdx.x % kWave;
   const int sr = ct.sig[cls * 4 + 0], st = ct.sig[cls * 4 + 1], sa = ct.sig[cls * 4 + 2], ss = ct.sig[cls * 4 + 3];
@@ -1951,10 +1950,11 @@
     }
     pc += __popcll(x.x) + __popcll(x.y);
     if (store) *(u64x2*)(dst + w) = x;
+    for (int i = 0; i < n_rows; ++i) *(u64x2*)(rows + (size_t)i * row_stride + w) = x;
   }
 #pragma unroll
   for (int off = 32; off > 0; off >>= 1) pc += __shfl_down(pc, off, kWave);
-  if (lane == 0) class_count[cls] = pc;
+  if (lane == 0 && counts) class_count[cls] = pc;
 }
 
 constexpr int kBandBlock = kBlock + kWave;
@@ -2044,14 +2044,6 @@
       run_band(std::integral_constant<int, kBandClasses>{});
     __syncthreads();
   }
-}
-__global__ __launch_bounds__(kBlock) void k_fix_rows(u64* __restrict__ out, const u64* __restrict__ class_rows, const int* __restrict__ rows,
-                                                     const int* __restrict__ slots, int n, int row_stride) {
-  typedef u64 u64x2 __attribute__((ext_vector_type(2)));
-  if ((int)blockIdx.x >= n) return;
-  const u64* src = class_rows + (size_t)slots[blockIdx.x] * row_stride;
-  u64* dst = out + (size_t)rows[blockIdx.x] * row_stride;
-  for (int w = threadIdx.x * 2; w < row_stride; w += 2 * kBlock) *(u64x2*)(dst + w) = *(const u64x2*)(src + w);
 }
 
 __global__ __launch_bounds__(kBlock) void k_decide(ClassTable ct, Planes ranked, int n_classes, int row_words, const int* __restrict__ perm,
```

Measured after the change: 41330 billion evals/s (median of 6 runs). 1.02x the previous value.
